# iwa-shi/CRDR

Measured on AMD Instinct MI355X. Metric: stage-3 training img/s at 256x256, higher is better.
Workload: dtype fp32; 1 GPU; config/crdr_stage_3.yaml -b 16: full GAN step (G + 5x CLIC21GVAE D + LPIPS-Alex, random-init weights), rate index cycled 0..4; global_batch=16, crop=256, parallelism=dp1

## Files before the change

crdr_amd/csrc/eltwise.hip:

```cpp

#include <algorithm>
#include <cmath>

#include "common.hpp"

namespace crdr {

struct EbwdArgs {
  crdr_ebwd_desc d;
  crdr_ebwd_io io;
  float* partial;
  int rows_per_block;
};

__global__ __launch_bounds__(256) void ebwd_kernel(const EbwdArgs p) {
  __shared__ float red[4][4][64];
  const int tx = threadIdx.x & 63, ty = threadIdx.x >> 6;
  const int f = p.d.flags, C = p.d.C;
  const int64_t r0 = (int64_t)blockIdx.x * p.rows_per_block;
  const int64_t r1 = r0 + p.rows_per_block < p.d.M ? r0 + p.rows_per_block : p.d.M;
  for (int c0 = 0; c0 < C; c0 += 64) {
    const int c = c0 + tx;
    float s0 = 0.f, s1 = 0.f, s2 = 0.f, s3 = 0.f;
    if (c < C) {
      const float sc = (f & CRDR_EPI_AFFINE) ? p.io.scale[c] : 1.f;
      const float sh = (f & CRDR_EPI_AFFINE) ? p.io.shift[c] : 0.f;
      const float v2 = (f & CRDR_EPI_VEC2) ? p.io.vec2[c] : 0.f;
      for (int64_t m = r0 + ty; m < r1; m += 4) {
        float g = p.io.dout[m * p.d.lddout + c];
        float o = (f & (CRDR_EPI_AFFINE | CRDR_EPI_RELU | CRDR_EPI_LRELU)) ? p.io.out[m * p.d.ldout + c] : 0.f;
        if (f & CRDR_EPI_AFFINE) {
          const float u = (o - sh) / sc;
          s2 += g * u;
          s3 += g;
          g *= sc;
          o = u;
        }
        if (f & CRDR_EPI_GATE) {
          const float sg = p.io.sig[m * p.d.ldg + c], tr = p.io.gt[m * p.d.ldg + c];
          p.io.gres[m * p.d.ldgres + c] = g;
          p.io.dgt[m * p.d.ldg + c] = g * sg;
          g = g * tr * sg * (1.f - sg);
        } else if ((f & CRDR_EPI_AFFINE) && (f & CRDR_EPI_RES)) {
          p.io.gres[m * p.d.ldgres + c] = g;
        }
        if (f & CRDR_EPI_VEC2) s1 += g;
        if (f & CRDR_EPI_RELU) g = (o - v2) > 0.f ? g : 0.f;
        if (f & CRDR_EPI_LRELU) g = o > 0.f ? g : 0.2f * g;
        if (p.io.dz) p.io.dz[m * p.d.lddz + c] = g;
        s0 += g;
      }
    }
    red[0][ty][tx] = s0; red[1][ty][tx] = s1; red[2][ty][tx] = s2; red[3][ty][tx] = s3;
    __syncthreads();
    if (ty == 0 && c < C) {
#pragma unroll
      for (int k = 0; k < 4; ++k)
        p.partial[((size_t)blockIdx.x * 4 + k) * C + c] = red[k][0][tx] + red[k][1][tx] + red[k][2][tx] + red[k][3][tx];
    }
    __syncthreads();
  }
}

__global__ __launch_bounds__(256) void ebwd_kernel_narrow(const EbwdArgs p) {
  __shared__ float red[16][256];
  const int f = p.d.flags, C = p.d.C, tid = threadIdx.x;
  const int64_t r0 = (int64_t)blockIdx.x * p.rows_per_block;
  const int64_t r1 = r0 + p.rows_per_block < p.d.M ? r0 + p.rows_per_block : p.d.M;
  float s[4][4];
  float sc[4], sh[4], v2[4];
#pragma unroll
  for (int c = 0; c < 4; ++c) {
    const bool live = c < C;
    sc[c] = (live && (f & CRDR_EPI_AFFINE)) ? p.io.scale[c] : 1.f;
    sh[c] = (live && (f & CRDR_EPI_AFFINE)) ? p.io.shift[c] : 0.f;
    v2[c] = (live && (f & CRDR_EPI_VEC2)) ? p.io.vec2[c] : 0.f;
#pragma unroll
    for (int k = 0; k < 4; ++k) s[k][c] = 0.f;
  }
  const bool need_out = f & (CRDR_EPI_AFFINE | CRDR_EPI_RELU | CRDR_EPI_LRELU);
  for (int64_t m = r0 + tid; m < r1; m += 256) {
#pragma unroll
    for (int c = 0; c < 4; ++c) {
      if (c >= C) continue;
      float g = p.io.dout[m * p.d.lddout + c];
      float o = need_out ? p.io.out[m * p.d.ldout + c] : 0.f;
      if (f & CRDR_EPI_AFFINE) {
// ... 190 lines not shown
      b += src[((size_t)sl * 2 + 1) * jb.cpad];
    }
    red[0][ty][tx] = a; red[1][ty][tx] = b;
    __syncthreads();
    if (ty == 0 && c < jb.C) {
      const float sa = ((red[0][0][tx] + red[0][1][tx]) + red[0][2][tx]) + red[0][3][tx];
      const float sb = ((red[1][0][tx] + red[1][1][tx]) + red[1][2][tx]) + red[1][3][tx];
      if (jb.out_pre) jb.out_pre[c] = jb.accumulate ? jb.out_pre[c] + sa : sa;
      if (jb.out_post) jb.out_post[c] = jb.accumulate ? jb.out_post[c] + sb : sb;
    }
    __syncthreads();
  }
}

static int ebwd_blocks(int64_t M, int* rpb) {
  int r = 64;
  while (cdiv64(M, r) > 512) r *= 2;
  *rpb = r;
  return (int)cdiv64(M, r);
}

__global__ __launch_bounds__(256) void affine_kernel(const float* x, int ldx, const float* scale, const float* shift,
                                                     float* y, int ldy, int64_t M, int C) {
  const int64_t total = M * C;
  for (int64_t e = blockIdx.x * 256ll + threadIdx.x; e < total; e += gridDim.x * 256ll) {
    const int64_t m = e / C;
    const int c = (int)(e - m * C);
    y[m * ldy + c] = x[m * ldx + c] * scale[c] + shift[c];
  }
}

__global__ __launch_bounds__(256) void add_affine_kernel(const float* a, int lda, const float* r, int ldr, const float* scale, const float* shift,
                                                         float* y, int ldy, int64_t M, int C4) {
  const int64_t total = M * C4;
  for (int64_t e = blockIdx.x * 256ll + threadIdx.x; e < total; e += gridDim.x * 256ll) {
    const int64_t m = e / C4;
    const int c = (int)(e - m * C4) * 4;
    f32x4 v = *reinterpret_cast<const f32x4*>(a + m * lda + c) + *reinterpret_cast<const f32x4*>(r + m * ldr + c);
    if (scale) v = v * *reinterpret_cast<const f32x4*>(scale + c) + *reinterpret_cast<const f32x4*>(shift + c);
    *reinterpret_cast<f32x4*>(y + m * ldy + c) = v;
  }
}

__global__ __launch_bounds__(256) void colsum_kernel(const float* x, int ldx, int64_t M, int C, float* partial,
                                                     int rows_per_block) {
  __shared__ float red[4][64];
  const int tx = threadIdx.x & 63, ty = threadIdx.x >> 6;
  const int64_t r0 = (int64_t)blockIdx.x * rows_per_block;
  const int64_t r1 = r0 + rows_per_block < M ? r0 + rows_per_block : M;
  for (int c0 = 0; c0 < C; c0 += 64) {
    const int c = c0 + tx;
    float s = 0.f;
    if (c < C)
      for (int64_t m = r0 + ty; m < r1; m += 4) s += x[m * ldx + c];
    red[ty][tx] = s;
    __syncthreads();
    if (ty == 0 && c < C) partial[(size_t)blockIdx.x * C + c] = red[0][tx] + red[1][tx] + red[2][tx] + red[3][tx];
    __syncthreads();
  }
}

__global__ __launch_bounds__(256) void colsum_kernel_v4(const float* x, int ldx, int64_t M, int C, float* partial,
                                                        int rows_per_block) {
  __shared__ f32x4 red[16][16];
  const int tx = threadIdx.x & 15, ty = threadIdx.x >> 4;
  const int c = blockIdx.y * 64 + tx * 4;
  const int64_t r0 = (int64_t)blockIdx.x * rows_per_block;
  const int64_t r1 = r0 + rows_per_block < M ? r0 + rows_per_block : M;
  f32x4 s = {0.f, 0.f, 0.f, 0.f};
  if (c < C)
    for (int64_t m = r0 + ty; m < r1; m += 16) s += *reinterpret_cast<const f32x4*>(x + m * ldx + c);
  red[ty][tx] = s;
  __syncthreads();
  if (threadIdx.x < 16 && c < C) {
    f32x4 a = red[0][tx];
#pragma unroll
    for (int r = 1; r < 16; ++r) a += red[r][tx];
    *reinterpret_cast<f32x4*>(partial + (size_t)blockIdx.x * C + c) = a;
  }
}

__device__ __forceinline__ float softplusf_(float w) { return w > 20.f ? w : log1pf(expf(w)); }

__global__ void interp_ca_params_kernel(const float* W, const float* B, int L, int C, float q, float* scale,
                                        float* shift) {
  const int c = blockIdx.x * blockDim.x + threadIdx.x;
  if (c >= C) return;
  const float lf = floorf(q);
  const float rf = fminf(lf + 1.f, (float)(L - 1));
  const float a = rf - q;
  const int l = (int)lf, r = (int)rf;
  const float w = W[l * C + c] * a + W[r * C + c] * (1.f - a);
  scale[c] = softplusf_(w);
  shift[c] = B ? B[l * C + c] * a + B[r * C + c] * (1.f - a) : 0.f;
}

__global__ void interp_ca_params_bwd_kernel(const float* W, int L, int C, float q, const float* dscale,
                                            const float* dshift, float* dW, float* dB) {
  const int c = blockIdx.x * blockDim.x + threadIdx.x;
  if (c >= C) return;
  const float lf = floorf(q);
  const float rf = fminf(lf + 1.f, (float)(L - 1));
  const float a = rf - q;
  const int l = (int)lf, r = (int)rf;
  const float w = W[l * C + c] * a + W[r * C + c] * (1.f - a);
  const float dw = dscale[c] * (w > 20.f ? 1.f : 1.f / (1.f + expf(-w)));
  dW[l * C + c] += dw * a;
  dW[r * C + c] += dw * (1.f - a);
  if (dB) {
    dB[l * C + c] += dshift[c] * a;
    dB[r * C + c] += dshift[c] * (1.f - a);
  }
}

__global__ __launch_bounds__(256) void lrp_kernel(const float* a, int lda, const float* z, int ldz, float* y, int ldy,
                                                  int64_t M, int C) {
  const int64_t total = M * C;
  for (int64_t e = blockIdx.x * 256ll + threadIdx.x; e < total; e += gridDim.x * 256ll) {
    const int64_t m = e / C;
    const int c = (int)(e - m * C);
    y[m * ldy + c] = a[m * lda + c] + 0.5f * tanhf(z[m * ldz + c]);
  }
}
__global__ __launch_bounds__(256) void lrp_bwd_kernel(const float* dy, int lddy, const float* z, int ldz, float* dz,
                                                      int lddz, int64_t M, int C) {
  const int64_t total = M * C;
  for (int64_t e = blockIdx.x * 256ll + threadIdx.x; e < total; e += gridDim.x * 256ll) {
    const int64_t m = e / C;
    const int c = (int)(e - m * C);
    const float t = tanhf(z[m * ldz + c]);
    dz[m * lddz + c] = dy[m * lddy + c] * 0.5f * (1.f - t * t);
  }
}

__global__ __launch_bounds__(256) void tanh_fwd_kernel(const float* x, int ldx, int64_t M, int C, int C4, float* y, int ldy) {
  const int64_t total = M * C4;
  for (int64_t e = blockIdx.x * 256ll + threadIdx.x; e < total; e += gridDim.x * 256ll) {
    const int64_t m = e / C4;
    const int c = (int)(e - m * C4) * 4;
    const f32x4 v = *reinterpret_cast<const f32x4*>(x + m * ldx + c);
    f32x4 o;
#pragma unroll
    for (int k = 0; k < 4; ++k) o[k] = c + k < C ? tanhf(v[k]) : 0.f;
    *reinterpret_cast<f32x4*>(y + m * ldy + c) = o;
  }
}
__global__ __launch_bounds__(256) void tanh_bwd_kernel(const float* y, int ldy, const float* dy, int lddy, int64_t M, int C, int C4,
                                                       float* dx, int lddx) {
  const int64_t total = M * C4;
  for (int64_t e = blockIdx.x * 256ll + threadIdx.x; e < total; e += gridDim.x * 256ll) {
    const int64_t m = e / C4;
    const int c = (int)(e - m * C4) * 4;
    const f32x4 t = *reinterpret_cast<const f32x4*>(y + m * ldy + c);
    const f32x4 g = *reinterpret_cast<const f32x4*>(dy + m * lddy + c);
    f32x4 o;
#pragma unroll
    for (int k = 0; k < 4; ++k) o[k] = c + k < C ? g[k] * (1.f - t[k] * t[k]) : 0.f;
    *reinterpret_cast<f32x4*>(dx + m * lddx + c) = o;
  }
}

__device__ __forceinline__ float block_sum_256(float v, float* red) {
#pragma unroll
  for (int o = 32; o > 0; o >>= 1) v += __shfl_down(v, o, 64);
  const int lane = threadIdx.x & 63, w = threadIdx.x >> 6;
  if (lane == 0) red[w] = v;
  __syncthreads();
  float r = red[0] + red[1] + red[2] + red[3];
  __syncthreads();
  return r;
}

enum { RED_SQDIFF = 0, RED_BCE = 1, RED_SQNORM = 2, RED_DOT = 3, RED_L1 = 4 };
template <int OP>
__global__ __launch_bounds__(256) void reduce_kernel(const float* a, const float* b, int64_t n, float target,
                                                     float* partial) {
  __shared__ float red[4];
  float s = 0.f;
  for (int64_t e = blockIdx.x * 256ll + threadIdx.x; e < n; e += gridDim.x * 256ll) {
    if (OP == RED_SQDIFF) { const float d = a[e] - b[e]; s += d * d; }
    if (OP == RED_L1) s += fabsf(a[e] - b[e]);
    if (OP == RED_SQNORM) { const float d = a[e]; s += d * d; }
    if (OP == RED_DOT) s += a[e] * b[e];
    if (OP == RED_BCE) {
      const float x = a[e] - b[e];
      s += fmaxf(x, 0.f) - x * target + log1pf(expf(-fabsf(x)));
    }
  }
  s = block_sum_256(s, red);
  if (threadIdx.x == 0) partial[blockIdx.x] = s;
}
__global__ __launch_bounds__(256) void reduce_final(const float* partial, int nb, float* out) {
  __shared__ float red[4];
  float s = 0.f;
  for (int e = threadIdx.x; e < nb; e += 256) s += partial[e];
  s = block_sum_256(s, red);
  if (threadIdx.x == 0) out[0] = s;
}
static int reduce_blocks(int64_t n) { return (int)std::min<int64_t>(std::max<int64_t>(cdiv64(n, 1024), 1), 1024); }

__global__ __launch_bounds__(256) void sqdiff_bwd_kernel(const float* a, const float* b, int64_t n, const float* g,
                                                         float gscale, float* da, float* db) {
  const float k = 2.f * gscale * (g ? g[0] : 1.f);
  for (int64_t e = blockIdx.x * 256ll + threadIdx.x; e < n; e += gridDim.x * 256ll) {
    const float d = (a[e] - b[e]) * k;
    if (da) da[e] = d;
    if (db) db[e] = -d;
  }
}
__global__ __launch_bounds__(256) void l1_bwd_kernel(const float* a, const float* b, int64_t n, const float* g, float gscale,
                                                     float* da, float* db) {
  const float k = gscale * (g ? g[0] : 1.f);
  for (int64_t e = blockIdx.x * 256ll + threadIdx.x; e < n; e += gridDim.x * 256ll) {
    const float x = a[e] - b[e];
    const float d = x > 0.f ? k : x < 0.f ? -k : 0.f;
    if (da) da[e] = d;
    if (db) db[e] = -d;
  }
}
__global__ __launch_bounds__(256) void bce_diff_bwd_kernel(const float* p, const float* q, int64_t n, float target,
                                                           const float* g, float gscale, float* dp, float* dq) {
  const float k = gscale * (g ? g[0] : 1.f);
  for (int64_t e = blockIdx.x * 256ll + threadIdx.x; e < n; e += gridDim.x * 256ll) {
    const float x = p[e] - q[e];
    const float d = (1.f / (1.f + expf(-x)) - target) * k;
    if (dp) dp[e] = d;
    if (dq) dq[e] = -d;
  }
}

__global__ __launch_bounds__(256) void adam_kernel(float* p, const float* g, float* m, float* v, int64_t n, float lr,
                                                   float b1, float b2, float eps, float bc1, float bc2_sqrt,
                                                   const float* sqnorm, float max_norm) {
  float clip = 1.f;
  if (sqnorm) {
    const float c = max_norm / (sqrtf(sqnorm[0]) + 1e-6f);
    clip = c < 1.f ? c : 1.f;
  }
  const float step_size = lr / bc1;
  for (int64_t e = blockIdx.x * 256ll + threadIdx.x; e < n; e += gridDim.x * 256ll) {
    const float gr = g[e] * clip;
    const float mm = m[e] + (gr - m[e]) * (1.f - b1);
    const float vv = v[e] * b2 + (1.f - b2) * gr * gr;
    m[e] = mm;
    v[e] = vv;
    const float denom = sqrtf(vv) / bc2_sqrt + eps;
    p[e] -= step_size * (mm / denom);
  }
}

__global__ __launch_bounds__(256) void adam_dyn_kernel(float* p, const float* g, float* m, float* v, int64_t n, float b1,
                                                       float b2, float eps, const float* dyn, const float* sqnorm,
                                                       float max_norm) {
  if (dyn[2] != 0.f) return;
  const float st = dyn[1];
  const float bc1 = 1.f - powf(b1, st), bc2_sqrt = sqrtf(1.f - powf(b2, st));
  float clip = 1.f;
  if (sqnorm) {
    const float c = max_norm / (sqrtf(sqnorm[0]) + 1e-6f);
    clip = c < 1.f ? c : 1.f;
  }
  const float step_size = dyn[0] / bc1;
  const bool vec = ((reinterpret_cast<uintptr_t>(p) | reinterpret_cast<uintptr_t>(g) | reinterpret_cast<uintptr_t>(m) | reinterpret_cast<uintptr_t>(v)) & 15) == 0;
  const int64_t n4 = vec ? n >> 2 : 0;
  for (int64_t e4 = blockIdx.x * 256ll + threadIdx.x; e4 < n4; e4 += gridDim.x * 256ll) {
    const f32x4 gv = reinterpret_cast<const f32x4*>(g)[e4], mv = reinterpret_cast<const f32x4*>(m)[e4], vv4 = reinterpret_cast<const f32x4*>(v)[e4];
    f32x4 pv = reinterpret_cast<const f32x4*>(p)[e4], mo, vo;
#pragma unroll
    for (int k = 0; k < 4; ++k) {
      const float gr = gv[k] * clip;
      const float mm = mv[k] + (gr - mv[k]) * (1.f - b1);
      const float vv = vv4[k] * b2 + (1.f - b2) * gr * gr;
      mo[k] = mm;
      vo[k] = vv;
      pv[k] -= step_size * (mm / (sqrtf(vv) / bc2_sqrt + eps));
    }
    reinterpret_cast<f32x4*>(m)[e4] = mo;
    reinterpret_cast<f32x4*>(v)[e4] = vo;
    reinterpret_cast<f32x4*>(p)[e4] = pv;
  }
  for (int64_t e = (n4 << 2) + blockIdx.x * 256ll + threadIdx.x; e < n; e += gridDim.x * 256ll) {
    const float gr = g[e] * clip;
    const float mm = m[e] + (gr - m[e]) * (1.f - b1);
    const float vv = v[e] * b2 + (1.f - b2) * gr * gr;
    m[e] = mm;
    v[e] = vv;
    p[e] -= step_size * (mm / (sqrtf(vv) / bc2_sqrt + eps));
  }
}

__global__ __launch_bounds__(256) void maxpool3s2_fwd_kernel(const float* x, float* y, int N, int H, int W, int C,
                                                             int OH, int OW) {
  const unsigned total = (unsigned)N * OH * OW * C;
  for (unsigned e = blockIdx.x * 256u + threadIdx.x; e < total; e += gridDim.x * 256u) {
    unsigned r = e / (unsigned)C;
    const int c = (int)(e - r * C);
    unsigned q = r / (unsigned)OW;
    const int ow = (int)(r - q * OW);
    const int n = (int)(q / (unsigned)OH), oh = (int)(q - (unsigned)n * OH);
    float best = -INFINITY;
    for (int i = 0; i < 3; ++i)
      for (int j = 0; j < 3; ++j) {
        const int ih = oh * 2 + i, iw = ow * 2 + j;
        if (ih < H && iw < W) best = fmaxf(best, x[(((int64_t)n * H + ih) * W + iw) * C + c]);
      }
    y[e] = best;
  }
}
__global__ __launch_bounds__(256) void maxpool3s2_bwd_kernel(const float* x, const float* dy, float* dx, int N, int H,
                                                             int W, int C, int OH, int OW) {
  const unsigned total = (unsigned)N * H * W * C;
  for (unsigned e = blockIdx.x * 256u + threadIdx.x; e < total; e += gridDim.x * 256u) {
    unsigned r = e / (unsigned)C;
    const int c = (int)(e - r * C);
    unsigned q = r / (unsigned)W;
    const int iw = (int)(r - q * W);
    const int n = (int)(q / (unsigned)H), ih = (int)(q - (unsigned)n * H);
    float acc = 0.f;
    for (int oh = (ih >= 2 ? (ih - 1) / 2 : 0); oh <= ih / 2 && oh < OH; ++oh)
      for (int ow = (iw >= 2 ? (iw - 1) / 2 : 0); ow <= iw / 2 && ow < OW; ++ow) {
        float best = -INFINITY; int bi = -1, bj = -1;
        for (int i = 0; i < 3; ++i)
          for (int j = 0; j < 3; ++j) {
            const int yy = oh * 2 + i, xx = ow * 2 + j;
            if (yy < H && xx < W) {
              const float v = x[(((int64_t)n * H + yy) * W + xx) * C + c];
              if (v > best) { best = v; bi = yy; bj = xx; }
            }
          }
        if (bi == ih && bj == iw) acc += dy[(((int64_t)n * OH + oh) * OW + ow) * C + c];
      }
    dx[e] = acc;
  }
}

__global__ __launch_bounds__(256) void lpips_layer_fwd_kernel(const float* f0, const float* f1, const float* lin,
                                                              int N, int HW, int C, float* partial) {
  __shared__ float red[4];
  const int lane = threadIdx.x & 63, w = threadIdx.x >> 6;
  const int n = blockIdx.y;
  float acc = 0.f;
  for (int px = blockIdx.x * 4 + w; px < HW; px += gridDim.x * 4) {
    const float* a = f0 + ((size_t)n * HW + px) * C;
    const float* b = f1 + ((size_t)n * HW + px) * C;
    float sa = 0.f, sb = 0.f;
    for (int c = lane; c < C; c += 64) { sa += a[c] * a[c]; sb += b[c] * b[c]; }
#pragma unroll
    for (int o = 32; o > 0; o >>= 1) { sa += __shfl_xor(sa, o, 64); sb += __shfl_xor(sb, o, 64); }
    const float ia = 1.f / (sqrtf(sa) + 1e-10f), ib = 1.f / (sqrtf(sb) + 1e-10f);
    float d = 0.f;
    for (int c = lane; c < C; c += 64) { const float t = a[c] * ia - b[c] * ib; d += lin[c] * t * t; }
#pragma unroll
    for (int o = 32; o > 0; o >>= 1) d += __shfl_xor(d, o, 64);
    acc += d;
  }
  if (lane == 0) red[w] = acc;
  __syncthreads();
  if (threadIdx.x == 0) partial[(size_t)n * gridDim.x + blockIdx.x] = red[0] + red[1] + red[2] + red[3];
}
__global__ void lpips_layer_final(const float* partial, int nb, int HW, float* out) {
  const int n = blockIdx.x;
  if (threadIdx.x == 0) {
    float s = 0.f;
    for (int b = 0; b < nb; ++b) s += partial[(size_t)n * nb + b];
    out[n] += s / (float)HW;
  }
}
__global__ __launch_bounds__(256) void lpips_layer_bwd_kernel(const float* f0, const float* f1, const float* lin,
                                                              int N, int HW, int C, const float* gout, float* df1) {
  const int lane = threadIdx.x & 63, w = threadIdx.x >> 6;
  const int n = blockIdx.y;
  const float g = gout[n] / (float)HW;
  for (int px = blockIdx.x * 4 + w; px < HW; px += gridDim.x * 4) {
    const float* a = f0 + ((size_t)n * HW + px) * C;
    const float* b = f1 + ((size_t)n * HW + px) * C;
    float* d = df1 + ((size_t)n * HW + px) * C;
    float sa = 0.f, sb = 0.f;
    for (int c = lane; c < C; c += 64) { sa += a[c] * a[c]; sb += b[c] * b[c]; }
#pragma unroll
    for (int o = 32; o > 0; o >>= 1) { sa += __shfl_xor(sa, o, 64); sb += __shfl_xor(sb, o, 64); }
    const float nb_ = sqrtf(sb);
    const float ia = 1.f / (sqrtf(sa) + 1e-10f), ib = 1.f / (nb_ + 1e-10f);
    float dot = 0.f;
    for (int c = lane; c < C; c += 64) {
      const float e = -2.f * g * lin[c] * (a[c] * ia - b[c] * ib);
      dot += e * b[c];
    }
#pragma unroll
    for (int o = 32; o > 0; o >>= 1) dot += __shfl_xor(dot, o, 64);
// ... 425 lines not shown
extern "C" int crdr_add_affine(const float* a, int lda, const float* r, int ldr, const float* scale, const float* shift, float* y, int ldy,
                               int64_t M, int C, crdr_stream_t s) {
  CRDR_REQUIRE(a && r && y && (!scale == !shift), "add_affine: null pointer (scale and shift come together)");
  CRDR_REQUIRE(M >= 0 && C > 0 && C % 4 == 0 && lda % 4 == 0 && ldr % 4 == 0 && ldy % 4 == 0 && lda >= C && ldr >= C && ldy >= C,
               "add_affine: C (%d) and the strides (%d, %d, %d) must be multiples of 4, the strides at least C", C, lda, ldr, ldy);
  CRDR_REQUIRE(((reinterpret_cast<uintptr_t>(a) | reinterpret_cast<uintptr_t>(r) | reinterpret_cast<uintptr_t>(y) |
                 reinterpret_cast<uintptr_t>(scale) | reinterpret_cast<uintptr_t>(shift)) & 15) == 0, "add_affine: operands must be 16-byte aligned");
  if (M == 0) return 0;
  hipLaunchKernelGGL(add_affine_kernel, dim3(grid_for(M * (C / 4))), dim3(256), 0, as_stream(s), a, lda, r, ldr, scale, shift, y, ldy, M, C / 4);
  CRDR_CHECK_LAUNCH("add_affine");
  return 0;
}

extern "C" size_t crdr_colsum_workspace(int64_t M, int C) {
  int rpb;
  return (size_t)ebwd_blocks(M, &rpb) * C * sizeof(float);
}
extern "C" int crdr_colsum(const float* x, int ldx, int64_t M, int C, float* out, int accumulate, void* ws,
                           size_t ws_bytes, crdr_stream_t s) {
  int rpb;
  const int nb = ebwd_blocks(M, &rpb);
  CRDR_REQUIRE(x && out && ws_bytes >= (size_t)nb * C * sizeof(float), "colsum: bad arguments");
  if (M > 0) {
    if ((C % 4 == 0) && (ldx % 4 == 0) && ((reinterpret_cast<uintptr_t>(x) & 15) == 0))
      hipLaunchKernelGGL(colsum_kernel_v4, dim3(nb, cdiv(C, 64)), dim3(256), 0, as_stream(s), x, ldx, M, C, (float*)ws, rpb);
    else
      hipLaunchKernelGGL(colsum_kernel, dim3(nb), dim3(256), 0, as_stream(s), x, ldx, M, C, (float*)ws, rpb);
    CRDR_CHECK_LAUNCH("colsum");
  }
  hipLaunchKernelGGL(colsum_final, dim3(cdiv(C, 16)), dim3(256), 0, as_stream(s), (const float*)ws, M > 0 ? nb : 0, 1,
                     C, out, accumulate, (float*)nullptr);
  CRDR_CHECK_LAUNCH("colsum_final");
  return 0;
}

extern "C" int crdr_colsum_slab_rows(void) { return kColsumSlab; }

extern "C" int crdr_colsum_finish_batched(const crdr_colsum_job* jobs, const int64_t* prefix_a, const int64_t* prefix_b,
                                          const int64_t* meta, float* scratch, crdr_stream_t s) {
  CRDR_REQUIRE(jobs && prefix_a && prefix_b && meta && scratch, "colsum_finish_batched: null pointer");
  hipLaunchKernelGGL(colsum_finish_a_kernel, dim3(4096), dim3(256), 0, as_stream(s), jobs, reinterpret_cast<const long long*>(prefix_a),
                     reinterpret_cast<const long long*>(meta), scratch);
  CRDR_CHECK_LAUNCH("colsum_finish_a_kernel");
  hipLaunchKernelGGL(colsum_finish_b_kernel, dim3(512), dim3(256), 0, as_stream(s), jobs, reinterpret_cast<const long long*>(prefix_b),
                     reinterpret_cast<const long long*>(meta), (const float*)scratch);
  CRDR_CHECK_LAUNCH("colsum_finish_b_kernel");
  return 0;
}

extern "C" int crdr_colsum_scatter(const float* x, int ldx, int64_t M, int C, int block, float* const* outs, int accumulate,
                                   void* ws, size_t ws_bytes, crdr_stream_t s) {
  int rpb;
  const int nb = ebwd_blocks(M, &rpb);
  CRDR_REQUIRE(x && outs && block > 0 && ws_bytes >= (size_t)nb * C * sizeof(float), "colsum_scatter: bad arguments");
  if (M > 0) {
    if ((C % 4 == 0) && (ldx % 4 == 0) && ((reinterpret_cast<uintptr_t>(x) & 15) == 0))
      hipLaunchKernelGGL(colsum_kernel_v4, dim3(nb, cdiv(C, 64)), dim3(256), 0, as_stream(s), x, ldx, M, C, (float*)ws, rpb);
    else
      hipLaunchKernelGGL(colsum_kernel, dim3(nb), dim3(256), 0, as_stream(s), x, ldx, M, C, (float*)ws, rpb);
    CRDR_CHECK_LAUNCH("colsum");
  }
  hipLaunchKernelGGL(colsum_final_scatter, dim3(cdiv(C, 16)), dim3(256), 0, as_stream(s), (const float*)ws, M > 0 ? nb : 0, C,
                     block, outs, accumulate);
  CRDR_CHECK_LAUNCH("colsum_final_scatter");
  return 0;
}

extern "C" int crdr_interp_ca_params(const float* W, const float* B, int L, int C, float q, float* scale,
                                     float* shift, crdr_stream_t s) {
  CRDR_REQUIRE(W && scale && shift, "interp_ca_params: null pointer");
  CRDR_REQUIRE(q >= 0.f && q <= (float)(L - 1), "interp_ca_params: rate_ind %f outside [0, %d]", q, L - 1);
  hipLaunchKernelGGL(interp_ca_params_kernel, dim3(cdiv(C, 64)), dim3(64), 0, as_stream(s), W, B, L, C, q, scale, shift);
  CRDR_CHECK_LAUNCH("interp_ca_params");
  return 0;
}
extern "C" int crdr_interp_ca_params_bwd(const float* W, int L, int C, float q, const float* dscale,
                                         const float* dshift, float* dW, float* dB, crdr_stream_t s) {
  CRDR_REQUIRE(W && dscale && dW, "interp_ca_params_bwd: null pointer");
  hipLaunchKernelGGL(interp_ca_params_bwd_kernel, dim3(cdiv(C, 64)), dim3(64), 0, as_stream(s), W, L, C, q, dscale,
                     dshift, dW, dB);
  CRDR_CHECK_LAUNCH("interp_ca_params_bwd");
  return 0;
}

extern "C" int crdr_lrp(const float* a, int lda, const float* z, int ldz, float* y, int ldy, int64_t M, int C,
                        crdr_stream_t s) {
  CRDR_REQUIRE(a && z && y, "lrp: null pointer");
  if (M * C == 0) return 0;
  hipLaunchKernelGGL(lrp_kernel, dim3(grid_for(M * C)), dim3(256), 0, as_stream(s), a, lda, z, ldz, y, ldy, M, C);
  CRDR_CHECK_LAUNCH("lrp");
  return 0;
}
extern "C" int crdr_lrp_bwd(const float* dy, int lddy, const float* z, int ldz, float* dz, int lddz, int64_t M, int C,
                            crdr_stream_t s) {
  CRDR_REQUIRE(dy && z && dz, "lrp_bwd: null pointer");
  if (M * C == 0) return 0;
  hipLaunchKernelGGL(lrp_bwd_kernel, dim3(grid_for(M * C)), dim3(256), 0, as_stream(s), dy, lddy, z, ldz, dz, lddz, M, C);
  CRDR_CHECK_LAUNCH("lrp_bwd");
  return 0;
}

static bool tanh_operand_ok(const float* p, int ld, int C) {
  return p && (reinterpret_cast<uintptr_t>(p) & 15) == 0 && ld % 4 == 0 && ld >= round_up(C, 4);
}
extern "C" int crdr_tanh_fwd(const float* x, int ldx, int64_t M, int C, float* y, int ldy, crdr_stream_t s) {
  CRDR_REQUIRE(M >= 0 && C > 0, "tanh_fwd: M (%lld) and C (%d) out of range", (long long)M, C);
  CRDR_REQUIRE(tanh_operand_ok(x, ldx, C) && tanh_operand_ok(y, ldy, C),
               "tanh_fwd: operands are 16-byte aligned, their strides multiples of 4 and at least C rounded up to 4");
  CRDR_REQUIRE(x != y || ldx == ldy, "tanh_fwd: in place needs one stride");
  if (M == 0) return 0;
  const int C4 = round_up(C, 4) / 4;
  hipLaunchKernelGGL(tanh_fwd_kernel, dim3(grid_for(M * C4)), dim3(256), 0, as_stream(s), x, ldx, M, C, C4, y, ldy);
  CRDR_CHECK_LAUNCH("tanh_fwd");
  return 0;
}
extern "C" int crdr_tanh_bwd(const float* y, int ldy, const float* dy, int lddy, int64_t M, int C, float* dx, int lddx, crdr_stream_t s) {
  CRDR_REQUIRE(M >= 0 && C > 0, "tanh_bwd: M (%lld) and C (%d) out of range", (long long)M, C);
  CRDR_REQUIRE(tanh_operand_ok(y, ldy, C) && tanh_operand_ok(dy, lddy, C) && tanh_operand_ok(dx, lddx, C),
               "tanh_bwd: operands are 16-byte aligned, their strides multiples of 4 and at least C rounded up to 4");
  CRDR_REQUIRE(dy != dx || lddy == lddx, "tanh_bwd: in place needs one stride");
  if (M == 0) return 0;
  const int C4 = round_up(C, 4) / 4;
  hipLaunchKernelGGL(tanh_bwd_kernel, dim3(grid_for(M * C4)), dim3(256), 0, as_stream(s), y, ldy, dy, lddy, M, C, C4, dx, lddx);
  CRDR_CHECK_LAUNCH("tanh_bwd");
  return 0;
}

struct BiasReluArgs {
  float* a;
  long long M;
  int ld, C, n;
  int c0[CRDR_MAX_GROUP];
  const float* bias[CRDR_MAX_GROUP];
};
__global__ __launch_bounds__(256) void bias_relu_slots_kernel(const BiasReluArgs p) {
  const int C4 = p.C >> 2;
  const long long per = p.M * C4, total = per * p.n;
  for (long long e = blockIdx.x * 256ll + threadIdx.x; e < total; e += gridDim.x * 256ll) {
    const int k = (int)(e / per);
    const long long r = e - k * per;
    const long long m = r / C4;
    const int c = (int)(r - m * C4) << 2;
    float* q = p.a + m * p.ld + p.c0[k] + c;
    const f32x4 v = *reinterpret_cast<const f32x4*>(q);
    const float* b = p.bias[k] + c;
    f32x4 o;
#pragma unroll
    for (int j = 0; j < 4; ++j) o[j] = fmaxf(v[j] + b[j], 0.f);
    *reinterpret_cast<f32x4*>(q) = o;
  }
}

extern "C" int crdr_bias_relu_slots(float* a, int ld, int64_t M, int C, int n, const int32_t* c0, const float* const* bias, crdr_stream_t s) {
  CRDR_REQUIRE(a && c0 && bias, "bias_relu_slots: null pointer");
  CRDR_REQUIRE(n >= 1 && n <= CRDR_MAX_GROUP && C % 4 == 0 && ld % 4 == 0 && (reinterpret_cast<uintptr_t>(a) & 15) == 0,
               "bias_relu_slots: %d slots of %d channels (ld %d)", n, C, ld);
  if (M * C == 0) return 0;
  BiasReluArgs p;
  p.a = a; p.M = M; p.ld = ld; p.C = C; p.n = n;
  for (int k = 0; k < n; ++k) {
    CRDR_REQUIRE(bias[k] && c0[k] % 4 == 0, "bias_relu_slots: slot %d misaligned", k);
    p.c0[k] = c0[k]; p.bias[k] = bias[k];
  }
  hipLaunchKernelGGL(bias_relu_slots_kernel, dim3(grid_for(M * (C / 4) * n)), dim3(256), 0, as_stream(s), p);
  CRDR_CHECK_LAUNCH("bias_relu_slots");
  return 0;
}

extern "C" size_t crdr_reduce_workspace(int64_t n) { return (size_t)reduce_blocks(n) * sizeof(float); }

template <int OP>
static int run_reduce(const float* a, const float* b, int64_t n, float target, float* out, void* ws, size_t ws_bytes,
                      crdr_stream_t s, const char* what) {
  const int nb = reduce_blocks(n);
  CRDR_REQUIRE(a && out && ws_bytes >= (size_t)nb * sizeof(float), "%s: bad arguments", what);
  hipLaunchKernelGGL(reduce_kernel<OP>, dim3(nb), dim3(256), 0, as_stream(s), a, b, n, target, (float*)ws);
  CRDR_CHECK_LAUNCH(what);
  hipLaunchKernelGGL(reduce_final, dim3(1), dim3(256), 0, as_stream(s), (const float*)ws, nb, out);
  CRDR_CHECK_LAUNCH(what);
  return 0;
}
extern "C" int crdr_spectral_norm_fwd(const float* w, int O, int K, float* u, float* v, int power_iter, float eps, float* w_out,
                                      float* sigma_out, void* ws, size_t ws_bytes, crdr_stream_t s) {
  CRDR_REQUIRE(w && u && v && w_out && sigma_out && ws, "spectral_norm_fwd: null pointer");
  CRDR_REQUIRE(ws_bytes >= (size_t)(O + K + 2) * sizeof(float), "spectral_norm_fwd: workspace too small");
  float* tv = (float*)ws;
  float* tu = tv + K;
  hipStream_t st = as_stream(s);
  if (power_iter) {
    hipLaunchKernelGGL(sn_wt_u_kernel, dim3(cdiv(K, 256)), dim3(256), 0, st, w, u, O, K, tv);
    hipLaunchKernelGGL(sn_normalize_kernel, dim3(1), dim3(1024), 0, st, tv, K, eps, v, 1, (float*)nullptr);
  }
  hipLaunchKernelGGL(sn_w_v_kernel, dim3(cdiv(O, 4)), dim3(256), 0, st, w, v, O, K, tu);
  hipLaunchKernelGGL(sn_normalize_kernel, dim3(1), dim3(1024), 0, st, tu, O, eps, u, power_iter ? 1 : 0, sigma_out);
  hipLaunchKernelGGL(sn_scale_kernel, dim3(grid_for((int64_t)O * K)), dim3(256), 0, st, w, sigma_out, (long long)O * K, w_out);
  CRDR_CHECK_LAUNCH("spectral_norm_fwd");
  return 0;
}

extern "C" int crdr_spectral_norm_bwd(const float* dw_sn, const float* w, const float* u, const float* v, const float* sigma,
                                      int O, int K, float* dw, void* ws, size_t ws_bytes, crdr_stream_t s) {
  CRDR_REQUIRE(dw_sn && w && u && v && sigma && dw && ws, "spectral_norm_bwd: null pointer");
  const int64_t n = (int64_t)O * K;
  const int nb = reduce_blocks(n);
  CRDR_REQUIRE(ws_bytes >= (size_t)(nb + 1) * sizeof(float), "spectral_norm_bwd: workspace too small");
  float* part = (float*)ws;
  float* dot = part + nb;
  hipStream_t st = as_stream(s);
  hipLaunchKernelGGL(reduce_kernel<RED_DOT>, dim3(nb), dim3(256), 0, st, dw_sn, w, n, 0.f, part);
  hipLaunchKernelGGL(reduce_final, dim3(1), dim3(256), 0, st, (const float*)part, nb, dot);
  hipLaunchKernelGGL(sn_bwd_kernel, dim3(grid_for(n)), dim3(256), 0, st, dw_sn, u, v, sigma, (const float*)dot, O, K, dw);
  CRDR_CHECK_LAUNCH("spectral_norm_bwd");
  return 0;
}

extern "C" int crdr_sqdiff_sum(const float* a, const float* b, int64_t n, float* out, void* ws, size_t ws_bytes,
                               crdr_stream_t s) {
  CRDR_REQUIRE(b, "sqdiff_sum: null pointer");
  return run_reduce<RED_SQDIFF>(a, b, n, 0.f, out, ws, ws_bytes, s, "sqdiff_sum");
}
extern "C" int crdr_l1_sum(const float* a, const float* b, int64_t n, float* out, void* ws, size_t ws_bytes, crdr_stream_t s) {
  CRDR_REQUIRE(b, "l1_sum: null pointer");
  return run_reduce<RED_L1>(a, b, n, 0.f, out, ws, ws_bytes, s, "l1_sum");
}
extern "C" int crdr_bce_diff_sum(const float* p, const float* q, int64_t n, float target, float* out, void* ws,
                                 size_t ws_bytes, crdr_stream_t s) {
  CRDR_REQUIRE(q, "bce_diff_sum: null pointer");
  return run_reduce<RED_BCE>(p, q, n, target, out, ws, ws_bytes, s, "bce_diff_sum");
}
extern "C" int crdr_sqnorm(const float* g, int64_t n, float* out, void* ws, size_t ws_bytes, crdr_stream_t s) {
  return run_reduce<RED_SQNORM>(g, nullptr, n, 0.f, out, ws, ws_bytes, s, "sqnorm");
}
extern "C" int crdr_sqdiff_bwd(const float* a, const float* b, int64_t n, const float* g, float gscale, float* da,
                               float* db, crdr_stream_t s) {
  CRDR_REQUIRE(a && b, "sqdiff_bwd: null pointer");
  if (n == 0) return 0;
  hipLaunchKernelGGL(sqdiff_bwd_kernel, dim3(grid_for(n)), dim3(256), 0, as_stream(s), a, b, n, g, gscale, da, db);
  CRDR_CHECK_LAUNCH("sqdiff_bwd");
  return 0;
}
extern "C" int crdr_l1_bwd(const float* a, const float* b, int64_t n, const float* g, float gscale, float* da, float* db,
                           crdr_stream_t s) {
  CRDR_REQUIRE(a && b, "l1_bwd: null pointer");
  if (n == 0) return 0;
  hipLaunchKernelGGL(l1_bwd_kernel, dim3(grid_for(n)), dim3(256), 0, as_stream(s), a, b, n, g, gscale, da, db);
  CRDR_CHECK_LAUNCH("l1_bwd");
  return 0;
}
extern "C" int crdr_bce_diff_bwd(const float* p, const float* q, int64_t n, float target, const float* g, float gscale,
                                 float* dp, float* dq, crdr_stream_t s) {
  CRDR_REQUIRE(p && q, "bce_diff_bwd: null pointer");
  if (n == 0) return 0;
  hipLaunchKernelGGL(bce_diff_bwd_kernel, dim3(grid_for(n)), dim3(256), 0, as_stream(s), p, q, n, target, g, gscale, dp, dq);
  CRDR_CHECK_LAUNCH("bce_diff_bwd");
  return 0;
}

extern "C" int crdr_adam_step(float* p, const float* g, float* m, float* v, int64_t n, float lr, float beta1,
                              float beta2, float eps, int step, const float* sqnorm, float max_norm, crdr_stream_t s) {
  CRDR_REQUIRE(p && g && m && v && step >= 1, "adam_step: bad arguments");
  if (n == 0) return 0;
  const float bc1 = 1.f - powf(beta1, (float)step);
  const float bc2_sqrt = sqrtf(1.f - powf(beta2, (float)step));
  hipLaunchKernelGGL(adam_kernel, dim3(grid_for(n)), dim3(256), 0, as_stream(s), p, g, m, v, n, lr, beta1, beta2, eps,
                     bc1, bc2_sqrt, sqnorm, max_norm);
  CRDR_CHECK_LAUNCH("adam_step");
  return 0;
}

extern "C" int crdr_adam_step_dyn(float* p, const float* g, float* m, float* v, int64_t n, float beta1, float beta2,
                                  float eps, const float* dyn, const float* sqnorm, float max_norm, crdr_stream_t s) {
  CRDR_REQUIRE(p && g && m && v && dyn, "adam_step_dyn: bad arguments");
  if (n == 0) return 0;
  hipLaunchKernelGGL(adam_dyn_kernel, dim3(grid_for(n)), dim3(256), 0, as_stream(s), p, g, m, v, n, beta1, beta2, eps, dyn,
                     sqnorm, max_norm);
  CRDR_CHECK_LAUNCH("adam_step_dyn");
  return 0;
}

extern "C" int crdr_maxpool3s2_fwd(const float* x, float* y, int N, int H, int W, int C, crdr_stream_t s) {
  CRDR_REQUIRE(x && y && H >= 3 && W >= 3, "maxpool: bad arguments");
  CRDR_REQUIRE((long long)N * H * W * C < (1ll << 31), "maxpool: %lld elements (32-bit element index)", (long long)N * H * W * C);
  const int OH = (H - 3) / 2 + 1, OW = (W - 3) / 2 + 1;
  hipLaunchKernelGGL(maxpool3s2_fwd_kernel, dim3(grid_for((int64_t)N * OH * OW * C)), dim3(256), 0, as_stream(s), x, y, N,
                     H, W, C, OH, OW);
  CRDR_CHECK_LAUNCH("maxpool_fwd");
  return 0;
}
extern "C" int crdr_maxpool3s2_bwd(const float* x, const float* dy, float* dx, int N, int H, int W, int C,
                                   crdr_stream_t s) {
  CRDR_REQUIRE(x && dy && dx && H >= 3 && W >= 3, "maxpool_bwd: bad arguments");
  CRDR_REQUIRE((long long)N * H * W * C < (1ll << 31), "maxpool_bwd: %lld elements (32-bit element index)", (long long)N * H * W * C);
  const int OH = (H - 3) / 2 + 1, OW = (W - 3) / 2 + 1;
  hipLaunchKernelGGL(maxpool3s2_bwd_kernel, dim3(grid_for((int64_t)N * H * W * C)), dim3(256), 0, as_stream(s), x, dy, dx,
                     N, H, W, C, OH, OW);
  CRDR_CHECK_LAUNCH("maxpool_bwd");
  return 0;
}

extern "C" int crdr_lpips_layer_fwd(const float* f0, const float* f1, const float* lin, int N, int HW, int C,
                                    float* out, void* ws, size_t ws_bytes, crdr_stream_t s) {
  CRDR_REQUIRE(f0 && f1 && lin && out && ws, "lpips_layer_fwd: bad arguments");
  const int nb = std::min(cdiv(HW, 4), 64);
  CRDR_REQUIRE(ws_bytes >= (size_t)N * nb * sizeof(float), "lpips_layer_fwd: workspace too small");
  float* part = (float*)ws;
  hipLaunchKernelGGL(lpips_layer_fwd_kernel, dim3(nb, N), dim3(256), 0, as_stream(s), f0, f1, lin, N, HW, C, part);
  CRDR_CHECK_LAUNCH("lpips_layer_fwd");
  hipLaunchKernelGGL(lpips_layer_final, dim3(N), dim3(64), 0, as_stream(s), (const float*)part, nb, HW, out);
  CRDR_CHECK_LAUNCH("lpips_layer_final");
  return 0;
}
extern "C" int crdr_lpips_layer_bwd(const float* f0, const float* f1, const float* lin, int N, int HW, int C,
                                    const float* gout, float* df1, crdr_stream_t s) {
  CRDR_REQUIRE(f0 && f1 && lin && gout && df1, "lpips_layer_bwd: bad arguments");
  const int nb = std::min(cdiv(HW, 4), 256);
  hipLaunchKernelGGL(lpips_layer_bwd_kernel, dim3(nb, N), dim3(256), 0, as_stream(s), f0, f1, lin, N, HW, C, gout, df1);
  CRDR_CHECK_LAUNCH("lpips_layer_bwd");
  return 0;
}
```

crdr_amd/csrc/entropy.hip:

```cpp

#include <algorithm>
#include <cmath>

#include "common.hpp"

namespace crdr {

__device__ __forceinline__ float exp_neg_sq(float x) {
  const float kL2Ehi = 1.44269502162933349609375f, kL2Elo = 1.92596299112661746e-8f;
  const float s = x * x, slo = __builtin_fmaf(x, x, -s);
  const float ti = __builtin_rintf(s * kL2Ehi);
  float tf = __builtin_fmaf(s, kL2Ehi, -ti);
  tf = __builtin_fmaf(s, kL2Elo, tf);
  tf = __builtin_fmaf(slo, kL2Ehi, tf);
  return __builtin_ldexpf(__builtin_amdgcn_exp2f(-tf), -(int)ti);
}
__device__ __forceinline__ float erfcx_pos(float a) {
  const float q = (a - 2.f) * __builtin_amdgcn_rcpf(a + 2.f);
  float p = 6.807514774e-05f;
  p = __builtin_fmaf(p, q, 1.608403462e-04f);
  p = __builtin_fmaf(p, q, -3.709284118e-04f);
  p = __builtin_fmaf(p, q, -1.395805088e-03f);
  p = __builtin_fmaf(p, q, 1.230503218e-03f);
  p = __builtin_fmaf(p, q, 8.689252695e-03f);
  p = __builtin_fmaf(p, q, -8.024739103e-03f);
  p = __builtin_fmaf(p, q, -5.421199524e-02f);
  p = __builtin_fmaf(p, q, 1.640504971e-01f);
  p = __builtin_fmaf(p, q, -1.660310904e-01f);
  p = __builtin_fmaf(p, q, -9.276381574e-02f);
  p = __builtin_fmaf(p, q, 2.769783912e-01f);
  const float r = __builtin_amdgcn_rcpf(__builtin_fmaf(2.f, a, 1.f));
  return __builtin_fmaf(p, r, r);
}
__device__ __forceinline__ float gc_rs(float sg) {
  const float r0 = __builtin_amdgcn_rcpf(sg);
  return __builtin_fmaf(__builtin_fmaf(-sg, r0, 1.f), r0, r0) * 0.70710678118654752440f;
}
__device__ __forceinline__ float gc_lik(float a, float rs, float& e_lo, float& e_hi) {
  const float xh = fminf((a + 0.5f) * rs, 1e4f), xl = fminf(fmaxf((a - 0.5f) * rs, -1e4f), 1e4f);
  e_hi = exp_neg_sq(xh);
  e_lo = exp_neg_sq(xl);
  const float th = e_hi * erfcx_pos(xh), tl = e_lo * erfcx_pos(fabsf(xl));
  const float l = 0.5f * ((xl < 0.f ? 2.f - tl : tl) - th);
  return a != a ? a : l;
}
__device__ __forceinline__ float gc_floor(float l, float bound) { return l < bound ? bound : l; }

__device__ __forceinline__ float block_sum(float v, float* red) {
#pragma unroll
  for (int o = 32; o > 0; o >>= 1) v += __shfl_down(v, o, 64);
  const int lane = threadIdx.x & 63, w = threadIdx.x >> 6, nw = blockDim.x >> 6;
  __syncthreads();
  if (lane == 0) red[w] = v;
  __syncthreads();
  float r = 0.f;
  for (int i = 0; i < nw; ++i) r += red[i];
  return r;
}

struct GcArgs {
  crdr_gc_desc2 d;
  crdr_gc_io io;
};

__device__ __forceinline__ void philox4x32_10(unsigned c0, unsigned c1, unsigned c2, unsigned c3, unsigned k0, unsigned k1,
                                              unsigned out[4]) {
#pragma unroll
  for (int r = 0; r < 10; ++r) {
    const unsigned hi0 = __umulhi(0xD2511F53u, c0), lo0 = 0xD2511F53u * c0;
    const unsigned hi1 = __umulhi(0xCD9E8D57u, c2), lo1 = 0xCD9E8D57u * c2;
    const unsigned n0 = hi1 ^ c1 ^ k0, n2 = hi0 ^ c3 ^ k1;
    c0 = n0; c1 = lo1; c2 = n2; c3 = lo0;
    k0 += 0x9E3779B9u; k1 += 0xBB67AE85u;
  }
  out[0] = c0; out[1] = c1; out[2] = c2; out[3] = c3;
}
__device__ __forceinline__ float philox_uniform(const uint64_t* ph, unsigned long long idx) {
  const unsigned long long seed = ph[0], ctr = ph[1] + (idx >> 2);
  unsigned o[4];
  philox4x32_10((unsigned)ctr, (unsigned)(ctr >> 32), 0u, 0u, (unsigned)seed, (unsigned)(seed >> 32), o);
  const unsigned r = o[idx & 3];
  return (float)(r >> 8) * (1.0f / 16777216.0f) - 0.5f;
}

__device__ __forceinline__ float gc_noise(const GcArgs& p, size_t pix, int c) {
  if (p.io.noise) return p.io.noise[pix * p.d.ldnoise + c];
  return philox_uniform(p.io.philox, (unsigned long long)pix * p.d.Ctot + p.d.c0 + c);
}

__device__ __forceinline__ void gc_elem(const GcArgs& p, float yv, float m, float sraw, float u, bool noisy, bool want_q, float& q_plus_m,
                                        float& lq, float& ln, float& sn, float& sq) {
  const float sg = fmaxf(sraw, p.d.scale_bound);
  const float rs = gc_rs(sg);
  const float q = rintf(yv - m);
  q_plus_m = q + m;
  float e0, e1;
  if (want_q) {
    float l = gc_lik(fabsf(q), rs, e0, e1);
    l = gc_floor(l, p.d.likelihood_bound);
    lq = l;
    sq -= __builtin_amdgcn_logf(l);
  }
  if (noisy) {
    float l = gc_lik(fabsf(yv + u - m), rs, e0, e1);
    l = gc_floor(l, p.d.likelihood_bound);
    ln = l;
    sn -= __builtin_amdgcn_logf(l);
  }
}

template <bool VEC>
__global__ __launch_bounds__(256) void gauss_cond_fwd_kernel(const GcArgs p, float* part) {
  __shared__ float red[16];
  const int n = blockIdx.y, C = p.d.C;
  const int per_img = p.d.HW * C;
  const bool noisy = p.io.noise || p.io.philox;
  const bool want_q = p.io.lik_quant || p.io.bits_quant;
  float sn = 0.f, sq = 0.f;
  if (VEC) {
    const int C4 = C >> 2;
    for (int e4 = blockIdx.x * 256 + threadIdx.x; e4 < (per_img >> 2); e4 += gridDim.x * 256) {
      const int px = e4 / C4, c = (e4 - px * C4) << 2;
      const size_t pix = (size_t)n * p.d.HW + px;
      const float4 yv = *reinterpret_cast<const float4*>(p.io.y + pix * p.d.ldy + c);
      const float4 mv = *reinterpret_cast<const float4*>(p.io.mu + pix * p.d.ldmu + c);
      const float4 sv = *reinterpret_cast<const float4*>(p.io.sigma + pix * p.d.ldsigma + c);
      float u[4] = {0.f, 0.f, 0.f, 0.f};
      if (p.io.noise) {
        const float4 nv = *reinterpret_cast<const float4*>(p.io.noise + pix * p.d.ldnoise + c);
        u[0] = nv.x; u[1] = nv.y; u[2] = nv.z; u[3] = nv.w;
      } else if (p.io.philox) {
        const unsigned long long idx = (unsigned long long)pix * p.d.Ctot + p.d.c0 + c;
        const unsigned long long seed = p.io.philox[0], ctr = p.io.philox[1] + (idx >> 2);
        unsigned o[4];
        philox4x32_10((unsigned)ctr, (unsigned)(ctr >> 32), 0u, 0u, (unsigned)seed, (unsigned)(seed >> 32), o);
#pragma unroll
        for (int j = 0; j < 4; ++j) u[j] = (float)(o[j] >> 8) * (1.0f / 16777216.0f) - 0.5f;
      }
      const float ya[4] = {yv.x, yv.y, yv.z, yv.w}, ma[4] = {mv.x, mv.y, mv.z, mv.w}, sa[4] = {sv.x, sv.y, sv.z, sv.w};
      float qm[4], lq[4], ln[4];
#pragma unroll
      for (int j = 0; j < 4; ++j) gc_elem(p, ya[j], ma[j], sa[j], u[j], noisy, want_q, qm[j], lq[j], ln[j], sn, sq);
      const float4 qv = make_float4(qm[0], qm[1], qm[2], qm[3]);
      if (p.io.yhat) *reinterpret_cast<float4*>(p.io.yhat + pix * p.d.ldyhat + c) = qv;
      if (p.io.yhat2) *reinterpret_cast<float4*>(p.io.yhat2 + pix * p.d.ldyhat2 + c) = qv;
      if (p.io.lik_quant) *reinterpret_cast<float4*>(p.io.lik_quant + pix * p.d.ldlik + c) = make_float4(lq[0], lq[1], lq[2], lq[3]);
      if (p.io.lik_noisy && noisy) *reinterpret_cast<float4*>(p.io.lik_noisy + pix * p.d.ldlik + c) = make_float4(ln[0], ln[1], ln[2], ln[3]);
    }
  } else {
    for (int e = blockIdx.x * 256 + threadIdx.x; e < per_img; e += gridDim.x * 256) {
      const int px = e / C, c = e - px * C;
      const size_t pix = (size_t)n * p.d.HW + px;
      float qm, lq = 0.f, ln = 0.f;
      gc_elem(p, p.io.y[pix * p.d.ldy + c], p.io.mu[pix * p.d.ldmu + c], p.io.sigma[pix * p.d.ldsigma + c],
              noisy ? gc_noise(p, pix, c) : 0.f, noisy, want_q, qm, lq, ln, sn, sq);
      if (p.io.yhat) p.io.yhat[pix * p.d.ldyhat + c] = qm;
      if (p.io.yhat2) p.io.yhat2[pix * p.d.ldyhat2 + c] = qm;
      if (p.io.lik_quant) p.io.lik_quant[pix * p.d.ldlik + c] = lq;
      if (p.io.lik_noisy && noisy) p.io.lik_noisy[pix * p.d.ldlik + c] = ln;
    }
  }
  sn = block_sum(sn, red);
  sq = block_sum(sq, red);
  if (threadIdx.x == 0) {
    if (part) {
      float* o = part + ((size_t)n * gridDim.x + blockIdx.x) * 2;
      o[0] = sn; o[1] = sq;
    } else {
      if (p.io.bits_noisy && noisy) p.io.bits_noisy[n] += sn;
      if (p.io.bits_quant) p.io.bits_quant[n] += sq;
    }
  }
}

__global__ __launch_bounds__(256) void gauss_cond_finish_kernel(const float* part, int B, float* bits_noisy, float* bits_quant) {
  __shared__ float red[16];
  const int n = blockIdx.x;
  float sn = 0.f, sq = 0.f;
  for (int b = threadIdx.x; b < B; b += 256) {
    const float2 v = *reinterpret_cast<const float2*>(part + ((size_t)n * B + b) * 2);
    sn += v.x; sq += v.y;
  }
  sn = block_sum(sn, red);
  sq = block_sum(sq, red);
  if (threadIdx.x == 0) {
    if (bits_noisy) bits_noisy[n] += sn;
    if (bits_quant) bits_quant[n] += sq;
  }
}

__device__ __forceinline__ void gc_elem_bwd(const GcArgs& p, float yv, float m, float sraw, float u, float gb, float ste, float& gy_out,
                                            float& gmu, float& gsig) {
  const float inv_ln2 = 1.4426950408889634f;
  const float sg = fmaxf(sraw, p.d.scale_bound);
  const float dlt = yv + u - m;
  const float a = fabsf(dlt), sgn = dlt > 0.f ? 1.f : (dlt < 0.f ? -1.f : 0.f);
  const float rs = gc_rs(sg), inv_sg = rs * 1.41421356237309504880f;
  const float zu = (0.5f - a) * inv_sg, zl = (-0.5f - a) * inv_sg;
  float e_lo, e_hi;
  const float lraw = gc_lik(a, rs, e_lo, e_hi);
  const float l = gc_floor(lraw, p.d.likelihood_bound);
  const float glik = gb * (-inv_ln2 / l);
  const float graw = (lraw < p.d.likelihood_bound && glik >= 0.f) ? 0.f : glik;
  const float pu = 0.39894228040143267794f * e_lo, pl = 0.39894228040143267794f * e_hi;
  const float dl_da = (pl - pu) * inv_sg;
  const float dl_dsg = (zl * pl - zu * pu) * inv_sg;
  const float gy = graw * dl_da * sgn;
  const float gsg = graw * dl_dsg;
  gsig = (sraw < p.d.scale_bound && gsg >= 0.f) ? 0.f : gsg;
  gy_out = gy + ste;
  gmu = -gy;
}

template <bool VEC>
__global__ __launch_bounds__(256) void gauss_cond_bwd_kernel(const GcArgs p) {
  const int C = p.d.C;
  const int per_img = p.d.HW * C;
  const int64_t total = (int64_t)p.d.N * per_img;
  if (VEC) {
    const int C4 = C >> 2;
    for (int64_t e4 = blockIdx.x * 256ll + threadIdx.x; e4 < (total >> 2); e4 += gridDim.x * 256ll) {
      const size_t pix = (size_t)(e4 / C4);
      const int c = (int)(e4 - (int64_t)pix * C4) << 2;
      const int n = (int)(pix / p.d.HW);
      const float4 yv = *reinterpret_cast<const float4*>(p.io.y + pix * p.d.ldy + c);
      const float4 mv = *reinterpret_cast<const float4*>(p.io.mu + pix * p.d.ldmu + c);
      const float4 sv = *reinterpret_cast<const float4*>(p.io.sigma + pix * p.d.ldsigma + c);
      float4 dv = make_float4(0.f, 0.f, 0.f, 0.f);
      if (p.io.dyhat) dv = *reinterpret_cast<const float4*>(p.io.dyhat + pix * p.d.lddyhat + c);
      float u[4];
      if (p.io.noise) {
        const float4 nv = *reinterpret_cast<const float4*>(p.io.noise + pix * p.d.ldnoise + c);
        u[0] = nv.x; u[1] = nv.y; u[2] = nv.z; u[3] = nv.w;
      } else {
        const unsigned long long idx = (unsigned long long)pix * p.d.Ctot + p.d.c0 + c;
        const unsigned long long seed = p.io.philox[0], ctr = p.io.philox[1] + (idx >> 2);
        unsigned o[4];
        philox4x32_10((unsigned)ctr, (unsigned)(ctr >> 32), 0u, 0u, (unsigned)seed, (unsigned)(seed >> 32), o);
#pragma unroll
        for (int j = 0; j < 4; ++j) u[j] = (float)(o[j] >> 8) * (1.0f / 16777216.0f) - 0.5f;
      }
      const float gb = p.io.gbits[n];
      const float ya[4] = {yv.x, yv.y, yv.z, yv.w}, ma[4] = {mv.x, mv.y, mv.z, mv.w}, sa[4] = {sv.x, sv.y, sv.z, sv.w};
      const float da[4] = {dv.x, dv.y, dv.z, dv.w};
      float gy[4], gm[4], gs[4];
#pragma unroll
      for (int j = 0; j < 4; ++j) gc_elem_bwd(p, ya[j], ma[j], sa[j], u[j], gb, da[j], gy[j], gm[j], gs[j]);
      *reinterpret_cast<float4*>(p.io.dy + pix * p.d.ldgrad + c) = make_float4(gy[0], gy[1], gy[2], gy[3]);
      *reinterpret_cast<float4*>(p.io.dmu + pix * p.d.ldgrad + c) = make_float4(gm[0], gm[1], gm[2], gm[3]);
      *reinterpret_cast<float4*>(p.io.dsigma + pix * p.d.ldgrad + c) = make_float4(gs[0], gs[1], gs[2], gs[3]);
    }
    return;
  }
  for (int64_t e = blockIdx.x * 256ll + threadIdx.x; e < total; e += gridDim.x * 256ll) {
    const int n = (int)(e / per_img);
    const size_t pix = (size_t)(e / C);
    const int c = (int)(e - (int64_t)pix * C);
    const float ste = p.io.dyhat ? p.io.dyhat[pix * p.d.lddyhat + c] : 0.f;
    float gy, gm, gs;
    gc_elem_bwd(p, p.io.y[pix * p.d.ldy + c], p.io.mu[pix * p.d.ldmu + c], p.io.sigma[pix * p.d.ldsigma + c], gc_noise(p, pix, c),
                p.io.gbits[n], ste, gy, gm, gs);
    p.io.dy[pix * p.d.ldgrad + c] = gy;
    p.io.dmu[pix * p.d.ldgrad + c] = gm;
    p.io.dsigma[pix * p.d.ldgrad + c] = gs;
  }
}

__global__ __launch_bounds__(256) void philox_uniform_kernel(const uint64_t* ph, int64_t M, int C, int Ctot, int c0, float* out, int ld) {
  const int64_t total = M * C;
  for (int64_t e = blockIdx.x * 256ll + threadIdx.x; e < total; e += gridDim.x * 256ll) {
    const int64_t pix = e / C;
// ... 139 lines not shown
    const float l = fmaxf(lraw, bound);
    const float glik = gbits[n] * (-inv_ln2 / l);
    const float graw = (lraw >= bound || glik < 0.f) ? glik : 0.f;
    const float sd = D > 0.f ? 1.f : (D < 0.f ? -1.f : 0.f);
    const float gu = graw * sd * A * (1.f - A) * s;
    const float gl = -graw * sd * B * (1.f - B) * s;
    float dx = eb_logits_bwd(P, v + 0.5f, Tu, gu, g);
    dx += eb_logits_bwd(P, v - 0.5f, Tl, gl, g);
    dz[idx] = dx + (dzhat ? dzhat[idx] : 0.f);
  }
  const int lane = threadIdx.x & 63, w = threadIdx.x >> 6;
#pragma unroll
  for (int i = 0; i < CRDR_EB_PARAMS; ++i) {
    float v = g[i];
#pragma unroll
    for (int o = 32; o > 0; o >>= 1) v += __shfl_down(v, o, 64);
    if (lane == 0) red[w][i] = v;
  }
  __syncthreads();
  if (threadIdx.x < CRDR_EB_PARAMS) {
    const int i = threadIdx.x;
    dparams[(size_t)c * CRDR_EB_PARAMS + i] = red[0][i] + red[1][i] + red[2][i] + red[3][i];
  }
}

__global__ __launch_bounds__(1024) void bits_kernel(const float* lik, int per_img, float* bits) {
  __shared__ float red[16];
  const int n = blockIdx.x;
  float s = 0.f;
  for (int e = threadIdx.x; e < per_img; e += blockDim.x) s -= logf(lik[(size_t)n * per_img + e]);
  s = block_sum(s, red);
  if (threadIdx.x == 0) bits[n] += s * 1.4426950408889634f;
}

__global__ __launch_bounds__(256) void eb_quantile_kernel(const float* quantiles, const float* params,
                                                          const float* target, int C, float* loss, float* dq) {
  __shared__ float red[16];
  float acc = 0.f;
  for (int e = threadIdx.x; e < C * 3; e += blockDim.x) {
    const int c = e / 3, j = e - c * 3;
    EbParams P;
    eb_load(params + (size_t)c * CRDR_EB_PARAMS, P);
    EbTape T;
    float g[CRDR_EB_PARAMS];
#pragma unroll
    for (int i = 0; i < CRDR_EB_PARAMS; ++i) g[i] = 0.f;
    const float x = quantiles[e];
    const float d = eb_logits(P, x, T) - target[j];
    const float sgn = d > 0.f ? 1.f : (d < 0.f ? -1.f : 0.f);
    acc += fabsf(d);
    dq[e] = eb_logits_bwd(P, x, T, sgn, g);
  }
  acc = block_sum(acc, red);
  if (threadIdx.x == 0) loss[0] = acc;
}

}

using namespace crdr;

extern "C" int crdr_eb_quantile_loss(const float* quantiles, const float* params, const float* target, int C,
                                     float* loss, float* dquantiles, crdr_stream_t s) {
  CRDR_REQUIRE(quantiles && params && target && loss && dquantiles, "eb_quantile_loss: null pointer");
  hipLaunchKernelGGL(eb_quantile_kernel, dim3(1), dim3(256), 0, as_stream(s), quantiles, params, target, C, loss,
                     dquantiles);
  CRDR_CHECK_LAUNCH("eb_quantile_loss");
  return 0;
}

static void gc_fill_defaults(crdr_gc_desc2& d) {
  if (!d.ldnoise) d.ldnoise = d.C;
  if (!d.ldlik) d.ldlik = d.C;
  if (!d.ldgrad) d.ldgrad = d.C;
  if (!d.Ctot) d.Ctot = d.C;
}

static int gc_blocks(const crdr_gc_desc2* d) {
  const long long per_img = (long long)d->HW * d->C;
  return (int)std::max<long long>(1, std::min<long long>(cdiv64(per_img, 1024), 2048));
}

extern "C" size_t crdr_gauss_cond_fwd_workspace(const crdr_gc_desc2* d) {
  if (!d) return 0;
  return (size_t)d->N * gc_blocks(d) * 2 * sizeof(float);
}

extern "C" int crdr_gauss_cond_fwd2(const crdr_gc_desc2* d, const crdr_gc_io* io, crdr_stream_t s) {
  CRDR_REQUIRE(d && io && io->y && io->mu && io->sigma, "gauss_cond_fwd: null input");
  GcArgs a;
  a.d = *d; a.io = *io;
  gc_fill_defaults(a.d);
  const long long per_img = (long long)d->HW * d->C;
  if (per_img == 0 || d->N == 0) return 0;
  CRDR_REQUIRE(per_img < (1ll << 31), "gauss_cond_fwd: %lld elements per image", per_img);
  auto al16 = [](const void* q) { return (reinterpret_cast<uintptr_t>(q) & 15) == 0; };
  const crdr_gc_desc2& g = a.d;
  const bool vec = g.C % 4 == 0 && g.ldy % 4 == 0 && g.ldmu % 4 == 0 && g.ldsigma % 4 == 0 && g.Ctot % 4 == 0 && g.c0 % 4 == 0 &&
                   al16(io->y) && al16(io->mu) && al16(io->sigma) && (!io->noise || (g.ldnoise % 4 == 0 && al16(io->noise))) &&
                   (!io->yhat || (g.ldyhat % 4 == 0 && al16(io->yhat))) && (!io->yhat2 || (g.ldyhat2 % 4 == 0 && al16(io->yhat2))) &&
                   ((!io->lik_noisy && !io->lik_quant) || (g.ldlik % 4 == 0 && al16(io->lik_noisy) && al16(io->lik_quant)));
  int B = gc_blocks(d);
  float* part = io->ws;
  if (!part || io->ws_bytes < crdr_gauss_cond_fwd_workspace(d) || !(io->bits_noisy || io->bits_quant)) {
    part = nullptr;
    if (io->bits_noisy || io->bits_quant) B = 1;
  }
  if (vec)
    hipLaunchKernelGGL(gauss_cond_fwd_kernel<true>, dim3(B, d->N), dim3(256), 0, as_stream(s), a, part);
  else
    hipLaunchKernelGGL(gauss_cond_fwd_kernel<false>, dim3(B, d->N), dim3(256), 0, as_stream(s), a, part);
  CRDR_CHECK_LAUNCH("gauss_cond_fwd");
  if (part) {
    const bool noisy = io->noise || io->philox;
    hipLaunchKernelGGL(gauss_cond_finish_kernel, dim3(d->N), dim3(256), 0, as_stream(s), part, B, noisy ? io->bits_noisy : nullptr,
                       io->bits_quant);
    CRDR_CHECK_LAUNCH("gauss_cond_finish");
  }
  return 0;
}

extern "C" int crdr_gauss_cond_bwd2(const crdr_gc_desc2* d, const crdr_gc_io* io, crdr_stream_t s) {
  CRDR_REQUIRE(d && io && io->y && io->mu && io->sigma && (io->noise || io->philox) && io->gbits && io->dy && io->dmu && io->dsigma,
               "gauss_cond_bwd: null pointer");
  GcArgs a;
  a.d = *d; a.io = *io;
  gc_fill_defaults(a.d);
  const int64_t total = (int64_t)d->N * d->HW * d->C;
  if (total == 0) return 0;
  auto al16 = [](const void* q) { return (reinterpret_cast<uintptr_t>(q) & 15) == 0; };
  const crdr_gc_desc2& g = a.d;
  const bool vec = g.C % 4 == 0 && g.ldy % 4 == 0 && g.ldmu % 4 == 0 && g.ldsigma % 4 == 0 && g.ldgrad % 4 == 0 && g.Ctot % 4 == 0 &&
                   g.c0 % 4 == 0 && al16(io->y) && al16(io->mu) && al16(io->sigma) && al16(io->dy) && al16(io->dmu) && al16(io->dsigma) &&
                   (!io->noise || (g.ldnoise % 4 == 0 && al16(io->noise))) && (!io->dyhat || (g.lddyhat % 4 == 0 && al16(io->dyhat)));
  const int nb = (int)std::min<int64_t>(cdiv64(vec ? total / 4 : total, 256), 4096);
  if (vec)
    hipLaunchKernelGGL(gauss_cond_bwd_kernel<true>, dim3(nb), dim3(256), 0, as_stream(s), a);
  else
    hipLaunchKernelGGL(gauss_cond_bwd_kernel<false>, dim3(nb), dim3(256), 0, as_stream(s), a);
  CRDR_CHECK_LAUNCH("gauss_cond_bwd");
  return 0;
}

__global__ __launch_bounds__(256) void gauss_symbols_kernel(const float* y, int ldy, const float* mu, int ldmu, const float* sigma,
                                                            int ldsg, const float* table, int levels, float bound, int N, int HW,
                                                            int C, int* sym, int* idx) {
  __shared__ float st[256];
  if (idx)
    for (int i = threadIdx.x; i < levels; i += 256) st[i] = table[i];
  __syncthreads();
  const long long total = (long long)N * C * HW;
  for (long long e = blockIdx.x * 256ll + threadIdx.x; e < total; e += gridDim.x * 256ll) {
    const int px = (int)(e % HW);
    const long long r = e / HW;
    const int c = (int)(r % C), n = (int)(r / C);
    const size_t pix = (size_t)n * HW + px;
    if (sym) sym[e] = (int)rintf(y[pix * ldy + c] - mu[pix * ldmu + c]);
    if (idx) {
      const float s = fmaxf(sigma[pix * ldsg + c], bound);
      int k = 0;
      for (int i = 0; i < levels - 1; ++i) k += (s > st[i]) ? 1 : 0;
      idx[e] = k;
    }
  }
}

extern "C" int crdr_gauss_symbols(const float* y, int ldy, const float* mu, int ldmu, const float* sigma, int ldsigma,
                                  const float* scale_table, int levels, float scale_bound, int N, int HW, int C, int32_t* symbols,
                                  int32_t* indexes, crdr_stream_t s) {
  CRDR_REQUIRE((!symbols || (y && mu)) && (!indexes || (sigma && scale_table)) && levels >= 1 && levels <= 256, "gauss_symbols: bad arguments");
  const long long total = (long long)N * C * HW;
  if (total == 0) return 0;
  hipLaunchKernelGGL(gauss_symbols_kernel, dim3((int)std::min<long long>(cdiv64(total, 256), 8192)), dim3(256), 0, as_stream(s), y, ldy, mu,
                     ldmu, sigma, ldsigma, scale_table, levels, scale_bound, N, HW, C, symbols, indexes);
  CRDR_CHECK_LAUNCH("gauss_symbols");
  return 0;
}

__global__ void philox_fork_kernel(uint64_t* state, uint64_t* call, unsigned long long inc) {
  call[0] = state[0];
  call[1] = state[1];
  state[1] += inc;
}

extern "C" int crdr_philox_fork(uint64_t* state, uint64_t* call, uint64_t inc, crdr_stream_t s) {
  CRDR_REQUIRE(state && call, "philox_fork: null pointer");
  hipLaunchKernelGGL(philox_fork_kernel, dim3(1), dim3(1), 0, as_stream(s), state, call, (unsigned long long)inc);
  CRDR_CHECK_LAUNCH("philox_fork");
  return 0;
}

extern "C" int crdr_philox_uniform(const uint64_t* philox, int N, int HW, int C, int Ctot, int c0, float* out, int ld,
                                   crdr_stream_t s) {
  CRDR_REQUIRE(philox && out, "philox_uniform: null pointer");
  const int64_t M = (int64_t)N * HW, total = M * C;
  if (total == 0) return 0;
// ... 60 lines not shown
```

crdr_amd/hip/functional.py:

```python
from __future__ import annotations

import ctypes as C
from typing import Optional, Tuple

import torch

from . import lib as L
from . import ops, packs

def grad_slot(p: torch.Tensor) -> torch.Tensor:
    if p.grad is None:
        p.grad = torch.zeros_like(p, memory_format=torch.contiguous_format)
    return p.grad


class ConvSpec:

    def __init__(self, in_ch, out_ch, k, stride, pad, transposed=False, out_pad=0):
        self.in_ch, self.out_ch, self.k = in_ch, out_ch, (k, k) if isinstance(k, int) else tuple(k)
        self.stride, self.pad, self.transposed, self.out_pad = stride, pad, transposed, out_pad
        self._packs = {}
        self.smallc = (not transposed) and in_ch <= 4
        self.smallc_dgrad = transposed and out_ch <= 4

# ... 225 lines not shown
            and x.shape[3] == 1 and x.shape[0] <= 16 and vec2 is None and res is None and affine is None and gate is None
            and act in (None, "relu") and weight.is_contiguous()):
        return _SmallLinear.apply(x, weight, bias, act == "relu")
    scale, shift = affine if affine is not None else (None, None)
    gx, gt = gate if gate is not None else (None, None)
    return _FusedConv.apply(x, weight, bias, vec2, res, scale, shift, gx, gt, spec, act, return_wgrad)


class _SpectralNorm(torch.autograd.Function):

    @staticmethod
    def forward(ctx, w_orig, u, v, training: bool, out_buf: torch.Tensor, eps: float):
        lib = L.load()
        ops._require_gpu(w_orig)
        o, k = w_orig.shape[0], w_orig.numel() // w_orig.shape[0]
        sigma = torch.empty(1, dtype=torch.float32, device=w_orig.device)
        ws, wsn = ops.workspace((o + k + 2) * 4, w_orig.device)
        L.check(lib.crdr_spectral_norm_fwd(w_orig.data_ptr(), o, k, u.data_ptr(), v.data_ptr(), int(training), float(eps),
                                           out_buf.data_ptr(), sigma.data_ptr(), ws, wsn, ops._stream()), "spectral_norm_fwd")
        ctx.save_for_backward(w_orig, u.clone() if training else u, v.clone() if training else v, sigma)
        return out_buf.detach()

    @staticmethod
    def backward(ctx, dw_sn):
        w_orig, u, v, sigma = ctx.saved_tensors
        lib = L.load()
        o, k = w_orig.shape[0], w_orig.numel() // w_orig.shape[0]
        g = grad_slot(w_orig)
        nb = lib.crdr_reduce_workspace(o * k) + 16
        ws, wsn = ops.workspace(nb, w_orig.device)
        L.check(lib.crdr_spectral_norm_bwd(dw_sn.contiguous().data_ptr(), w_orig.data_ptr(), u.data_ptr(), v.data_ptr(),
                                           sigma.data_ptr(), o, k, g.data_ptr(), ws, wsn, ops._stream()), "spectral_norm_bwd")
        return None, None, None, None, None, None


def spectral_norm_weight(w_orig, u, v, training: bool, out_buf: torch.Tensor, eps: float = 1e-12):
    return _SpectralNorm.apply(w_orig, u, v, training, out_buf, eps)


class _InterpCaVectors(torch.autograd.Function):
    @staticmethod
    def forward(ctx, W, B, q: float):
        lib = L.load()
        Lv, Cc = W.shape[0], W.shape[2]
        scale = torch.empty(Cc, dtype=torch.float32, device=W.device)
        shift = torch.empty(Cc, dtype=torch.float32, device=W.device)
        L.check(lib.crdr_interp_ca_params(W.data_ptr(), None if B is None else B.data_ptr(), Lv, Cc, float(q),
                                          scale.data_ptr(), shift.data_ptr(), ops._stream()), "interp_ca_params")
        ctx.q, ctx.has_b = float(q), B is not None
        ctx.B = B
        ctx.save_for_backward(W)
        return scale, shift

    @staticmethod
    def backward(ctx, dscale, dshift):
        (W,) = ctx.saved_tensors
        lib = L.load()
        Lv, Cc = W.shape[0], W.shape[2]
        direct = W.is_leaf and (ctx.B is None or ctx.B.is_leaf)
        if direct:
            dW = grad_slot(W) if ctx.needs_input_grad[0] else None
            dB = grad_slot(ctx.B) if (ctx.has_b and ctx.needs_input_grad[1]) else None
        else:
            dW = torch.zeros_like(W)
            dB = torch.zeros_like(W) if ctx.has_b else None
        if dW is not None or dB is not None:
            scratch = None
            if dW is None:
                scratch = dW = torch.zeros_like(W)
            L.check(lib.crdr_interp_ca_params_bwd(W.data_ptr(), Lv, Cc, ctx.q, dscale.contiguous().data_ptr(),
                                                  dshift.contiguous().data_ptr(), dW.data_ptr(),
                                                  None if dB is None else dB.data_ptr(), ops._stream()), "interp_ca_params_bwd")
            if scratch is not None:
                dW = None
        if direct:
            return None, None, None
        return dW, dB, None


def interp_ca_vectors(W, B, q: float):
    return _InterpCaVectors.apply(W, B, float(q))


class _Affine(torch.autograd.Function):
    @staticmethod
    def forward(ctx, x, scale, shift):
        lib = L.load()
        x, ld = ops.nhwc(x)
        n, c, h, w = x.shape
        y = ops.empty_nhwc(n, c, h, w, x.device)
        L.check(lib.crdr_affine(x.data_ptr(), ld, scale.data_ptr(), shift.data_ptr(), y.data_ptr(), ops.ld_for(c), n * h * w, c,
                                ops._stream()), "affine")
        ctx.save_for_backward(y, scale, shift)
        return y

    @staticmethod
    def backward(ctx, dy):
        y, scale, shift = ctx.saved_tensors
        dz, _, _, cs = ops.epilogue_bwd(dy, y, L.EPI_AFFINE, scale=scale, shift=shift)
        return dz, cs[2], cs[3]


def affine(x, scale, shift):
    return _Affine.apply(x, scale, shift)


class _AddAffine(torch.autograd.Function):

    @staticmethod
    def forward(ctx, a, r, scale, shift):
        lib = L.load()
        a, lda = ops.nhwc(a)
        r, ldr = ops.nhwc(r)
        if a.shape != r.shape:
            raise L.CrdrHipError(f"add_affine: operands of shapes {tuple(a.shape)} and {tuple(r.shape)}")
        n, c, h, w = a.shape
        y = ops.empty_nhwc(n, c, h, w, a.device)
        L.check(lib.crdr_add_affine(a.data_ptr(), lda, r.data_ptr(), ldr, ops._p(scale), ops._p(shift), y.data_ptr(), ops.ld_for(c), n * h * w, c,
                                    ops._stream()), "add_affine")
        ctx.save_for_backward(*((y, scale, shift) if scale is not None else ()))
        return y

    @staticmethod
    def backward(ctx, dy):
        if not ctx.saved_tensors:
            return dy, dy, None, None
        y, scale, shift = ctx.saved_tensors
        dz, _, _, cs = ops.epilogue_bwd(dy, y, L.EPI_AFFINE, scale=scale, shift=shift)
        return dz, dz, cs[2], cs[3]


def add_affine(a, r, affine: Optional[Tuple[torch.Tensor, torch.Tensor]] = None):
    scale, shift = affine if affine is not None else (None, None)
    return _AddAffine.apply(a, r, scale, shift)


class _PixelShuffle(torch.autograd.Function):

    @staticmethod
    def forward(ctx, x):
        lib = L.load()
        x, ldx = ops.nhwc(x)
        n, c4, h, w = x.shape
        if c4 % 4 != 0:
            raise L.CrdrHipError(f"pixel_shuffle: {c4} input channels are not a multiple of 4")
        c = c4 // 4
        y = ops.empty_nhwc(n, c, 2 * h, 2 * w, x.device)
        L.check(lib.crdr_pixel_shuffle_fwd(x.data_ptr(), ldx, n, h, w, c, y.data_ptr(), ops.ld_for(c), ops._stream()), "pixel_shuffle_fwd")
        ctx.in_shape = (n, c4, h, w)
        return y

    @staticmethod
    def backward(ctx, dy):
        lib = L.load()
        n, c4, h, w = ctx.in_shape
        dy, lddy = ops.nhwc(dy)
        dx = ops.empty_nhwc(n, c4, h, w, dy.device)
        L.check(lib.crdr_pixel_shuffle_bwd(dy.data_ptr(), lddy, n, h, w, c4 // 4, dx.data_ptr(), c4, ops._stream()), "pixel_shuffle_bwd")
        return dx


def pixel_shuffle(x):
    return _PixelShuffle.apply(x)


UPSAMPLE16_MODES = {"nearest": 0, "bilinear": 1, "bicubic": 2}
# ... 279 lines not shown
        return out

    @staticmethod
    def backward(ctx, g):
        fa, fb = ctx.saved_tensors
        lib = L.load()
        entry = _PAIR_SUMS[ctx.name][1]
        da = torch.empty_like(fa) if ctx.needs_input_grad[0] else None
        db = torch.empty_like(fb) if ctx.needs_input_grad[1] else None
        L.check(getattr(lib, "crdr_" + entry)(fa.data_ptr(), fb.data_ptr(), fa.numel(), *ctx.targs, g.contiguous().data_ptr(), 1.0,
                                              ops._p(da), ops._p(db), ops._stream()), entry)
        return _unflat(da, ctx.shapes[0], ctx.geom), _unflat(db, ctx.shapes[1], ctx.geom), None, None


def sqdiff_sum(a, b):
    return _PairSum.apply(a, b, "sqdiff_sum", None)


def l1_sum(a, b):
    return _PairSum.apply(a, b, "l1_sum", None)


def bce_diff_sum(p, q, target: float):
    return _PairSum.apply(p, q, "bce_diff_sum", float(target))


GAN_BCE, GAN_HINGE_D, GAN_HINGE_G = 0, 1, 2


class _GanLossSum(torch.autograd.Function):

    @staticmethod
    def forward(ctx, p, q, mask, kind, target, sgn, center):
        lib = L.load()
        fp = p.contiguous().reshape(-1)
        fq = None if q is None else q.contiguous().reshape(-1)
        fm = None if mask is None else mask.expand_as(p).contiguous().reshape(-1)
        if fq is not None and not center and fq.numel() != fp.numel():
            raise ValueError(f"gan_loss_sum: paired operands of {fp.numel()} and {fq.numel()} elements")
        if center and fq is None:
            raise ValueError("gan_loss_sum: center=True needs q")
        for t in (fp, fq, fm):
            if t is not None and (t.dtype != torch.float32 or t.device != p.device or not t.is_cuda):
                raise ValueError("gan_loss_sum: operands are float32 tensors on one GPU")
        d = L.GanLossDesc(n=fp.numel(), nq=0 if fq is None else fq.numel(), kind=int(kind), center=int(bool(center)),
                          target=float(target), sgn=float(sgn))
        out = torch.empty(1, dtype=torch.float32, device=p.device)
        stats = torch.empty(2, dtype=torch.float32, device=p.device)
        ws, wsn = ops.workspace(lib.crdr_gan_loss_workspace(d.n, d.nq), p.device)
        L.check(lib.crdr_gan_loss_fwd(C.byref(d), fp.data_ptr(), ops._p(fq), ops._p(fm), out.data_ptr(), stats.data_ptr(), ws, wsn,
                                      ops._stream()), "gan_loss_fwd")
        ctx.desc, ctx.has_q, ctx.has_mask = d, fq is not None, fm is not None
        ctx.shapes = (p.shape, None if q is None else q.shape)
        ctx.save_for_backward(fp, stats, *([fq] if fq is not None else []), *([fm] if fm is not None else []))
        return out

    @staticmethod
    def backward(ctx, g):
        lib = L.load()
        fp, stats, *rest = ctx.saved_tensors
        fq = rest.pop(0) if ctx.has_q else None
        fm = rest.pop(0) if ctx.has_mask else None
        d = ctx.desc
        dp = torch.empty_like(fp) if ctx.needs_input_grad[0] else None
        dq = torch.empty_like(fq) if (fq is not None and ctx.needs_input_grad[1]) else None
        ws, wsn = ops.workspace(lib.crdr_gan_loss_workspace(d.n, d.nq), fp.device)
        L.check(lib.crdr_gan_loss_bwd(C.byref(d), fp.data_ptr(), ops._p(fq), ops._p(fm), stats.data_ptr(), g.contiguous().data_ptr(), 1.0,
                                      ops._p(dp), ops._p(dq), ws, wsn, ops._stream()), "gan_loss_bwd")
        return (_unflat(dp, ctx.shapes[0], None), _unflat(dq, ctx.shapes[1], None), None, None, None, None, None)


def gan_loss_sum(p, q=None, *, kind: int, target: float = 0.0, sgn: float = 1.0, center: bool = False, mask=None):
    return _GanLossSum.apply(p, q, mask, int(kind), float(target), float(sgn), bool(center))


class _MaxPool3s2(torch.autograd.Function):
    @staticmethod
    def forward(ctx, x):
        lib = L.load()
        x = ops.dense_nhwc(x)
        n, c, h, w = x.shape
        oh, ow = (h - 3) // 2 + 1, (w - 3) // 2 + 1
        y = ops.empty_nhwc(n, c, oh, ow, x.device, ld=c)
        L.check(lib.crdr_maxpool3s2_fwd(x.data_ptr(), y.data_ptr(), n, h, w, c, ops._stream()), "maxpool_fwd")
        ctx.save_for_backward(x)
        return y

    @staticmethod
    def backward(ctx, dy):
        (x,) = ctx.saved_tensors
        lib = L.load()
        n, c, h, w = x.shape
        dy = ops.dense_nhwc(dy)
        dx = ops.empty_nhwc(n, c, h, w, x.device, ld=c)
        L.check(lib.crdr_maxpool3s2_bwd(x.data_ptr(), dy.data_ptr(), dx.data_ptr(), n, h, w, c, ops._stream()), "maxpool_bwd")
        return dx


def maxpool3s2(x):
    return _MaxPool3s2.apply(x)


class _LpipsLayer(torch.autograd.Function):

    @staticmethod
    def forward(ctx, f0, f1, lin):
        lib = L.load()
        f0, f1 = ops.dense_nhwc(f0), ops.dense_nhwc(f1)
        n, c, h, w = f0.shape
        out = torch.zeros(n, dtype=torch.float32, device=f0.device)
        ws, wsn = ops.workspace(n * 64 * 4, f0.device)
        L.check(lib.crdr_lpips_layer_fwd(f0.data_ptr(), f1.data_ptr(), lin.data_ptr(), n, h * w, c, out.data_ptr(), ws, wsn,
                                         ops._stream()), "lpips_layer_fwd")
        ctx.save_for_backward(f0, f1, lin)
        return out

    @staticmethod
    def backward(ctx, g):
        f0, f1, lin = ctx.saved_tensors
        lib = L.load()
        n, c, h, w = f0.shape
        df1 = ops.empty_nhwc(n, c, h, w, f0.device, ld=c)
        L.check(lib.crdr_lpips_layer_bwd(f0.data_ptr(), f1.data_ptr(), lin.data_ptr(), n, h * w, c, g.contiguous().data_ptr(),
                                         df1.data_ptr(), ops._stream()), "lpips_layer_bwd")
        return None, df1, None


def lpips_layer(f_real, f_fake, lin):
    return _LpipsLayer.apply(f_real, f_fake, lin)
```

crdr_amd/hip/lib.py:

```python
from __future__ import annotations

import ctypes as C
import os
import subprocess
import threading

_HERE = os.path.dirname(os.path.abspath(__file__))
CSRC_DIR = os.path.normpath(os.path.join(_HERE, "..", "csrc"))
LIB_PATH = os.environ.get("CRDR_HIP_LIB") or os.path.normpath(os.path.join(_HERE, "..", "_lib", "libcrdr_hip.so"))

c_float_p = C.POINTER(C.c_float)
c_void_p = C.c_void_p


class ConvDesc(C.Structure):
    _fields_ = [(n, C.c_int32) for n in (
        "N", "H", "W", "C", "OH", "OW", "OC", "kh", "kw", "stride", "pad", "transposed", "ldx", "ldy",
        "wrows", "wcols", "flags", "ldres", "ldg", "wlayout", "reserved", "ldpre", "ldmask")]


class ConvIO(C.Structure):
    _fields_ = [(n, c_void_p) for n in (
        "x", "w", "y", "bias", "vec2", "res", "scale", "shift", "gx", "gt", "sig", "pre", "mask", "cs")]


class ColsumJob(C.Structure):
    _fields_ = [("cs", c_void_p), ("out_pre", c_void_p), ("out_post", c_void_p)] + [(n, C.c_int32) for n in (
        "rows", "ld", "C", "accumulate", "nslab", "cpad")] + [("scratch_off", C.c_int64)]


class WgradDesc(C.Structure):
    _fields_ = [(n, C.c_int32) for n in (
        "N", "PH", "PW", "PC", "ldp", "QH", "QW", "QC", "ldq", "kh", "kw", "stride", "pad", "gI", "gJ",
        "accumulate", "algo")]


class EbwdDesc(C.Structure):
    _fields_ = [("M", C.c_int64)] + [(n, C.c_int32) for n in (
        "C", "flags", "lddout", "ldout", "lddz", "ldgres", "ldg")]


class WgradJob(C.Structure):
    _fields_ = [("slab", c_void_p), ("g", c_void_p)] + [(n, C.c_int32) for n in (
        "PC", "QC", "gI", "gJ", "T", "nsplit", "smallj", "accumulate", "gJtot", "reserved")]


class LinearGroup(C.Structure):
    _fields_ = [(n, c_void_p * 16) for n in ("w", "b", "y", "dy", "dw", "db")] + [("O", C.c_int32 * 16)]


class PackItem(C.Structure):
    _fields_ = [("src", c_void_p), ("dst", c_void_p)] + [(n, C.c_int32) for n in (
        "I", "J", "T", "rows", "cols", "mode", "srcJ", "dld")] + [("tstride", C.c_int64)]


class W4FilterItem(C.Structure):
    _fields_ = [("w", c_void_p * 16), ("u", c_void_p)] + [(n, C.c_int32) for n in (
        "G", "Cin", "Cout", "wrows", "wcols", "kchunks", "ntile", "nvar")] + [("widx", (C.c_int32 * 9) * 4), ("units", C.c_int64)]


class GdnDesc(C.Structure):
    _fields_ = [("M", C.c_int64)] + [(n, C.c_int32) for n in ("C", "ldx", "ldy", "inverse")] + [
        ("beta_min", C.c_float), ("reparam_offset", C.c_float)]


class ChannelNormDesc(C.Structure):
    _fields_ = [("M", C.c_int64)] + [(n, C.c_int32) for n in ("C", "ldx", "ldy", "ldres", "act")] + [
        ("slope", C.c_float), ("eps", C.c_float)]


class InstanceNormDesc(C.Structure):
    _fields_ = [("HW", C.c_int64)] + [(n, C.c_int32) for n in ("N", "C", "ldx", "ldy", "act")] + [("slope", C.c_float), ("eps", C.c_float)]


class GanLossDesc(C.Structure):
    _fields_ = [("n", C.c_int64), ("nq", C.c_int64), ("kind", C.c_int32), ("center", C.c_int32), ("target", C.c_float), ("sgn", C.c_float)]


class Upsample16Desc(C.Structure):
    _fields_ = [(n, C.c_int32) for n in ("N", "h", "w", "Cc", "ldi", "ldc", "ldo", "mode")]


class GcDesc2(C.Structure):
    _fields_ = [(n, C.c_int32) for n in ("N", "HW", "C", "ldy", "ldmu", "ldsigma", "ldyhat", "ldyhat2", "ldnoise", "ldlik",
                                         "ldgrad", "lddyhat", "Ctot", "c0")] + [
        ("scale_bound", C.c_float), ("likelihood_bound", C.c_float)]


class GcIO(C.Structure):
    _fields_ = [(n, c_void_p) for n in ("y", "mu", "sigma", "noise", "philox", "yhat", "yhat2", "lik_noisy", "lik_quant",
                                        "bits_noisy", "bits_quant", "gbits", "dyhat", "dy", "dmu", "dsigma", "ws")] + [
        ("ws_bytes", C.c_size_t)]


class EbwdIO(C.Structure):
    _fields_ = [(n, c_void_p) for n in (
        "dout", "out", "vec2", "scale", "shift", "gt", "sig", "dz", "gres", "dgt", "colsums", "dbias_accum")]


class GcDesc(C.Structure):
    _fields_ = [(n, C.c_int32) for n in ("N", "HW", "C", "ldy", "ldmu", "ldsigma", "ldyhat")] + [
        ("scale_bound", C.c_float), ("likelihood_bound", C.c_float)]


EPI_BIAS, EPI_RELU, EPI_LRELU, EPI_VEC2, EPI_RES, EPI_GATE, EPI_AFFINE, EPI_ACCUM = 1, 2, 4, 8, 16, 32, 64, 128
EPI_PREADD, EPI_RELUMASK, EPI_LRELUMASK, EPI_MASKOFF, EPI_COLSUM = 256, 512, 1024, 2048, 4096
CONV_NOSPLIT, CONV_BF16X3, WGRAD_BF16X3 = 8192, 16384, 1 << 16
CONV_BF16X6, WGRAD_BF16X6 = 32768, 1 << 17
WGRAD_SQUARE_Q = 1 << 18
MAX_GROUP = 16
EB_PARAMS = 58

_I, _I64, _F, _D, _P, _SZ = C.c_int, C.c_int64, C.c_float, C.c_double, c_void_p, C.c_size_t
SIGNATURES = {
    "crdr_last_error": (C.c_char_p, []),
    "crdr_version": (_I, []),
    "crdr_arch": (C.c_char_p, []),
    "crdr_profile_enable": (None, [_I]),
    "crdr_profile_read": (_I, [_I, C.POINTER(C.c_double), C.POINTER(C.c_double), C.POINTER(C.c_longlong)]),
    "crdr_conv2d_num_configs": (_I, []),
    "crdr_conv2d_num_stream_configs": (_I, []),
    "crdr_conv2d_num_wino_configs": (_I, []),
    "crdr_conv2d_wgrad_num_configs": (_I, []),
    "crdr_conv2d_wgrad_num_wino_configs": (_I, []),
    "crdr_conv2d_workspace": (_SZ, [C.POINTER(ConvDesc)]),
    "crdr_conv2d_choose_algo": (_I, [C.POINTER(ConvDesc), _I]),
    "crdr_conv2d": (_I, [C.POINTER(ConvDesc), C.POINTER(ConvIO), _P, _SZ, _P]),
    "crdr_conv2d_flops": (_D, [C.POINTER(ConvDesc)]),
    "crdr_conv2d_colsum_layout": (_I, [C.POINTER(ConvDesc), _I, C.POINTER(C.c_int), C.POINTER(C.c_int)]),
    "crdr_colsum_slab_rows": (_I, []),
    "crdr_colsum_finish_batched": (_I, [_P, _P, _P, _P, _P, _P]),
    "crdr_conv2d_grouped_workspace": (_SZ, [C.POINTER(ConvDesc), _I]),
    "crdr_conv2d_grouped": (_I, [C.POINTER(ConvDesc), _P, _I, _P, _SZ, _P]),
    "crdr_conv2d_filter_cache_bytes": (_SZ, [C.POINTER(ConvDesc), _I]),
    "crdr_conv2d_grouped_ex": (_I, [C.POINTER(ConvDesc), _P, _I, _P, _SZ, _P, _SZ, _I, _P]),
    "crdr_conv2d_filter_item": (_I, [C.POINTER(ConvDesc), _I, C.POINTER(W4FilterItem)]),
    "crdr_w4_filters_batched": (_I, [_P, _P, _P, _P]),
    "crdr_conv2d_wgrad_grouped_workspace": (_SZ, [C.POINTER(WgradDesc), _I]),
    "crdr_conv2d_wgrad_partial_grouped": (_I, [C.POINTER(WgradDesc), _P, _P, _P, _I, _P, _SZ, _P, _P]),
    "crdr_pack_weight_item": (_I, [C.POINTER(PackItem), _P]),
    "crdr_colsum_scatter": (_I, [_P, _I, _I64, _I, _I, _P, _I, _P, _SZ, _P]),
    "crdr_gauss_cond_fwd_workspace": (_SZ, [C.POINTER(GcDesc2)]),
    "crdr_gauss_cond_fwd2": (_I, [C.POINTER(GcDesc2), C.POINTER(GcIO), _P]),
    "crdr_gauss_cond_bwd2": (_I, [C.POINTER(GcDesc2), C.POINTER(GcIO), _P]),
    "crdr_gdn_workspace": (_SZ, [C.POINTER(GdnDesc), _I]),
    "crdr_gdn_fwd": (_I, [C.POINTER(GdnDesc), _P, _P, _P, _P, _P, _SZ, _P]),
    "crdr_gdn_bwd": (_I, [C.POINTER(GdnDesc), _P, _P, _P, _P, _I, _P, _I, _P, _P, _P, _SZ, _P]),
    "crdr_gdn_res_fwd": (_I, [C.POINTER(GdnDesc), _P, _P, _P, _P, _I, _P, _P, _SZ, _P]),
    "crdr_channel_norm_workspace": (_SZ, [C.POINTER(ChannelNormDesc)]),
    "crdr_channel_norm_fwd": (_I, [C.POINTER(ChannelNormDesc), _P, _P, _P, _P, _P, _P, _P]),
    "crdr_channel_norm_bwd": (_I, [C.POINTER(ChannelNormDesc), _P, _P, _P, _P, _P, _I, _P, _I, _P, _P, _P, _SZ, _P]),
    "crdr_instance_norm_workspace": (_SZ, [C.POINTER(InstanceNormDesc)]),
    "crdr_instance_norm_fwd": (_I, [C.POINTER(InstanceNormDesc), _P, _P, _P, _P, _P, _P, _SZ, _P]),
    "crdr_instance_norm_bwd": (_I, [C.POINTER(InstanceNormDesc), _P, _P, _P, _P, _P, _I, _P, _I, _P, _P, _P, _SZ, _P]),
    "crdr_reflect_pad_fwd": (_I, [_P, _I, _I, _I, _I, _I, _I, _I, _I, _I, _P, _I, _P]),
    "crdr_reflect_pad_bwd": (_I, [_P, _I, _I, _I, _I, _I, _I, _I, _I, _I, _P, _I, _P]),
    "crdr_pixel_shuffle_fwd": (_I, [_P, _I, _I, _I, _I, _I, _P, _I, _P]),
    "crdr_pixel_shuffle_bwd": (_I, [_P, _I, _I, _I, _I, _I, _P, _I, _P]),
    "crdr_upsample16_cat_workspace": (_SZ, [C.POINTER(Upsample16Desc)]),
    "crdr_upsample16_cat_fwd": (_I, [C.POINTER(Upsample16Desc), _P, _P, _P, _P]),
    "crdr_upsample16_cat_bwd": (_I, [C.POINTER(Upsample16Desc), _P, _P, _P, _P, _SZ, _P]),
    "crdr_gauss_symbols": (_I, [_P, _I, _P, _I, _P, _I, _P, _I, _F, _I, _I, _I, _P, _P, _P]),
    "crdr_philox_fork": (_I, [_P, _P, C.c_uint64, _P]),
    "crdr_philox_uniform": (_I, [_P, _I, _I, _I, _I, _I, _P, _I, _P]),
    "crdr_conv2d_wgrad_workspace": (_SZ, [C.POINTER(WgradDesc)]),
    "crdr_conv2d_wgrad": (_I, [C.POINTER(WgradDesc), _P, _P, _P, _P, _SZ, _P]),
    "crdr_conv2d_wgrad_partial": (_I, [C.POINTER(WgradDesc), _P, _P, _P, _P, _SZ, C.POINTER(WgradJob), _P]),
    "crdr_wgrad_reduce_batched": (_I, [_P, _P, _P, _P]),
    "crdr_pack_weight": (_I, [_P, _P, _I, _I, _I, _I, _I, _I, _P]),
    "crdr_pack_weights_batched": (_I, [_P, _P, _P, _P]),
    "crdr_epilogue_bwd_workspace": (_SZ, [C.POINTER(EbwdDesc)]),
    "crdr_epilogue_bwd": (_I, [C.POINTER(EbwdDesc), C.POINTER(EbwdIO), _P, _SZ, _P]),
    "crdr_col2im_rgb": (_I, [_P, _I, _I, _I, _I, _I, _I, _I, _I, _P, _P, _I, _I, _I, _I, _P]),
    "crdr_spectral_norm_fwd": (_I, [_P, _I, _I, _P, _P, _I, C.c_float, _P, _P, _P, _SZ, _P]),
    "crdr_spectral_norm_bwd": (_I, [_P, _P, _P, _P, _P, _I, _I, _P, _P, _SZ, _P]),
    "crdr_crop_flip_normalize": (_I, [_P, _P, _I, _I, _I, _P, _I, _P]),
    "crdr_linear_fwd": (_I, [_P, _I, _I, _I, _P, _P, _P, _I, _I, _I, _P]),
    "crdr_linear_bwd": (_I, [_P, _I, _I, _I, _P, _P, _I, _P, _I, _I, _P, _I, _P, _P, _P]),
    "crdr_linear_group_fwd": (_I, [_P, _I, _I, _I, _P, _I, _P]),
    "crdr_linear_group_bwd": (_I, [_P, _I, _I, _I, _P, _I, _P, _I, _P]),
    "crdr_affine": (_I, [_P, _I, _P, _P, _P, _I, _I64, _I, _P]),
    "crdr_colsum_workspace": (_SZ, [_I64, _I]),
    "crdr_colsum": (_I, [_P, _I, _I64, _I, _P, _I, _P, _SZ, _P]),
    "crdr_interp_ca_params": (_I, [_P, _P, _I, _I, _F, _P, _P, _P]),
    "crdr_interp_ca_params_bwd": (_I, [_P, _I, _I, _F, _P, _P, _P, _P, _P]),
    "crdr_bias_relu_slots": (_I, [_P, _I, _I64, _I, _I, _P, _P, _P]),
    "crdr_lrp": (_I, [_P, _I, _P, _I, _P, _I, _I64, _I, _P]),
    "crdr_lrp_bwd": (_I, [_P, _I, _P, _I, _P, _I, _I64, _I, _P]),
    "crdr_add_affine": (_I, [_P, _I, _P, _I, _P, _P, _P, _I, _I64, _I, _P]),
    "crdr_tanh_fwd": (_I, [_P, _I, _I64, _I, _P, _I, _P]),
    "crdr_tanh_bwd": (_I, [_P, _I, _P, _I, _I64, _I, _P, _I, _P]),
    "crdr_gauss_cond_fwd": (_I, [C.POINTER(GcDesc), _P, _P, _P, _P, _P, _P, _P, _P, _P, _P]),
    "crdr_gauss_cond_bwd": (_I, [C.POINTER(GcDesc), _P, _P, _P, _P, _P, _P, _I, _P, _P, _P, _P]),
    "crdr_entropy_bottleneck_fwd": (_I, [_P, _P, _P, _P, _I, _I, _I, _F, _P, _P, _P, _P]),
    "crdr_entropy_bottleneck_bwd": (_I, [_P, _P, _P, _I, _I, _I, _F, _P, _P, _P, _P, _P]),
    "crdr_eb_quantile_loss": (_I, [_P, _P, _P, _I, _P, _P, _P]),
    "crdr_reduce_workspace": (_SZ, [_I64]),
    "crdr_sqdiff_sum": (_I, [_P, _P, _I64, _P, _P, _SZ, _P]),
    "crdr_sqdiff_bwd": (_I, [_P, _P, _I64, _P, _F, _P, _P, _P]),
    "crdr_bce_diff_sum": (_I, [_P, _P, _I64, _F, _P, _P, _SZ, _P]),
    "crdr_bce_diff_bwd": (_I, [_P, _P, _I64, _F, _P, _F, _P, _P, _P]),
    "crdr_gan_loss_workspace": (_SZ, [_I64, _I64]),
    "crdr_gan_loss_fwd": (_I, [C.POINTER(GanLossDesc), _P, _P, _P, _P, _P, _P, _SZ, _P]),
    "crdr_gan_loss_bwd": (_I, [C.POINTER(GanLossDesc), _P, _P, _P, _P, _P, _F, _P, _P, _P, _SZ, _P]),
    "crdr_l1_sum": (_I, [_P, _P, _I64, _P, _P, _SZ, _P]),
    "crdr_l1_bwd": (_I, [_P, _P, _I64, _P, _F, _P, _P, _P]),
    "crdr_msssim_workspace": (_SZ, [_I, _I, _I, _I]),
    "crdr_msssim_fwd": (_I, [_P, _I, _P, _I, _I, _I, _I, _I, _F, _I, _P, _SZ, _I, _P, _P]),
    "crdr_msssim_bwd": (_I, [_P, _I, _P, _I, _I, _I, _I, _I, _P, _P, _P, _I, _P, _I, _P, _SZ, _P]),
    "crdr_sqnorm": (_I, [_P, _I64, _P, _P, _SZ, _P]),
    "crdr_adam_step": (_I, [_P, _P, _P, _P, _I64, _F, _F, _F, _F, _I, _P, _F, _P]),
    "crdr_adam_step_dyn": (_I, [_P, _P, _P, _P, _I64, _F, _F, _F, _P, _P, _F, _P]),
    "crdr_maxpool3s2_fwd": (_I, [_P, _P, _I, _I, _I, _I, _P]),
    "crdr_maxpool3s2_bwd": (_I, [_P, _P, _P, _I, _I, _I, _I, _P]),
    "crdr_lpips_layer_fwd": (_I, [_P, _P, _P, _I, _I, _I, _P, _P, _SZ, _P]),
    "crdr_lpips_layer_bwd": (_I, [_P, _P, _P, _I, _I, _I, _P, _P, _P]),
    "crdr_pmf_to_quantized_cdf": (_I, [_P, _I, _I, _P]),
    "crdr_rans_encode_with_indexes": (_I64, [_P, _P, _I64, _P, _I, _P, _P, _I, _P, _I64]),
    "crdr_rans_decoder_create": (_P, []),
    "crdr_rans_decoder_destroy": (None, [_P]),
    "crdr_rans_decoder_set_stream": (_I, [_P, _P, _I64]),
    "crdr_rans_decoder_decode_stream": (_I, [_P, _P, _I64, _P, _I, _P, _P, _I, _P]),
    "crdr_rans_decode_with_indexes": (_I, [_P, _I64, _P, _I64, _P, _I, _P, _P, _I, _P]),
}


class CrdrHipError(RuntimeError):
    pass


def build(force: bool = False, jobs: int = 6) -> str:
    if force:
        subprocess.run(["make", "-C", CSRC_DIR, "clean"], check=True, stdout=subprocess.DEVNULL)
    r = subprocess.run(["make", "-C", CSRC_DIR, f"-j{jobs}"], stdout=subprocess.PIPE, stderr=subprocess.STDOUT, text=True)
    if r.returncode != 0:
        raise CrdrHipError("building libcrdr_hip.so failed:\n" + r.stdout[-4000:])
    return LIB_PATH


_lock = threading.Lock()
_lib = None


def load():
    global _lib
    if _lib is not None:
        return _lib
    with _lock:
        if _lib is not None:
            return _lib
        if not os.path.exists(LIB_PATH):
            raise CrdrHipError(
                f"{LIB_PATH} not found: the HIP extension is required (run `python -c 'import __graft_entry__ as g; "
                "g.build()'` or `make -C crdr_amd/csrc`). There is no CPU fallback.")
        lib = C.CDLL(LIB_PATH)
        for name, (res, args) in SIGNATURES.items():
            fn = getattr(lib, name)
            fn.restype = res
            fn.argtypes = args
        _lib = lib
    return _lib


def check(rc, what: str = ""):
    if rc is not None and rc < 0:
        msg = load().crdr_last_error().decode("utf-8", "replace")
        raise CrdrHipError(f"{what}: rc={rc}: {msg}")
    return rc
```

crdr_amd/hip/ops.py:

```python
from __future__ import annotations

import contextlib
import ctypes as C
import os
from typing import Optional, Tuple

import torch

from . import lib as L
from . import packs, tune
from .batched import BumpArena, JobTable, SiteTables, _capturing, _require_gpu, _stream

_ws_cache = {}
_ws_keep = []
_ws_max = 0

AUTOTUNE = False
FORCED_CONV_ALGO = 0
MATRIX_BF16X3 = False
MATRIX_BF16X6 = False


def _matrix_mode() -> int:
    return 2 if MATRIX_BF16X6 else (1 if MATRIX_BF16X3 else 0)
# ... 92 lines not shown
    return ids


def _conv_trial(lib, d, ios, G: int, device, colsum: bool, trial_out):
    if trial_out is not None:
        tio, res_t, reset = ios, trial_out, None
    else:
        span = (d.N * d.OH * d.OW - 1) * d.ldy + d.OC
        res_t, reset = tune.scratch(G * span + 64, device)
        tio = (L.ConvIO * G)()
        C.memmove(tio, ios, C.sizeof(tio))
        for g in range(G):
            tio[g].y = res_t.data_ptr() + 4 * g * span
            if ios[g].pre == ios[g].y:
                tio[g].pre = tio[g].y
            if ios[g].res == ios[g].y:
                tio[g].res = tio[g].y
    keep, cost = [], 0.0

    def run(a):
        nonlocal cost
        d.reserved = a
        if colsum:
            try:
                _, _, nf = _colsum_layout(lib, d, G)
            except L.CrdrHipError:
                return False
            keep[:] = [torch.empty(G * nf, dtype=torch.float32, device=device)]
            for g in range(G):
                tio[g].cs = keep[0].data_ptr() + 4 * g * nf
        ok, cost = _tune_conv_launch(lib, d, tio, G, device)
        return ok
    return run, (lambda: res_t), reset, (lambda: cost)


def _wgrad_trial(lib, d, G: int, pa, qa, device, whole: bool):
    gsize = d.gI * d.gJ * d.kh * d.kw
    tmp = torch.zeros(G * gsize + 64, dtype=torch.float32, device=device)
    ta = (C.c_void_p * G)(*[tmp.data_ptr() + 4 * g * gsize for g in range(G)])
    jobs_t = (L.WgradJob * G)()
    d, slab = L.WgradDesc.from_buffer_copy(d), 0
    d.accumulate = 0 if whole else d.accumulate

    def run(a):
        nonlocal slab
        d.algo = _wa(a)
        nb = lib.crdr_conv2d_wgrad_grouped_workspace(C.byref(d), G)
        if nb == 0 or nb > (2 << 30):
            return False
        slab = nb
        w_, wn_ = workspace(nb, device)
        if whole:
            return lib.crdr_conv2d_wgrad(C.byref(d), pa[0], qa[0], ta[0], w_, wn_, _stream()) == 0
        return lib.crdr_conv2d_wgrad_partial_grouped(C.byref(d), pa, qa, ta, G, w_, wn_, jobs_t, _stream()) == 0
    if whole:
        return run, (lambda: tmp), None, None

    def result():
        reduce_jobs_now(jobs_t, device)
        return tmp
    return run, result, tmp.zero_, (lambda: slab / 3.8e9)


PROFILE = None


def _prof_begin():
    if PROFILE is None:
        return None
    e = torch.cuda.Event(enable_timing=True)
    e.record()
    return e


def _prof_end(kind: str, flops: float, e0, label: str = "", nbytes: float = 0.0) -> None:
    if e0 is None:
        return
    e1 = torch.cuda.Event(enable_timing=True)
    e1.record()
    PROFILE.setdefault(kind, []).append((flops, e0, e1, label, nbytes))


_WS_HEAD = 4 * 16384


def _ws_fit(key, device, need: Optional[int]) -> torch.Tensor:
    size = max(int(_ws_max * 1.25), 1 << 20)
    buf = _ws_cache.get(key)
    if buf is None or buf.numel() < (size if need is None else need):
        if need is not None and torch.cuda.is_current_stream_capturing():
            raise L.CrdrHipError("workspace must be reserved before graph capture (ops.reserve_workspace); "
                                 f"need {need} bytes, have {0 if buf is None else buf.numel()}")
        if buf is not None:
            _ws_keep.append(buf)
        buf = _ws_cache[key] = torch.zeros(size, dtype=torch.uint8, device=device)
    return buf


def workspace(nbytes: int, device, conv: bool = False) -> Tuple[int, int]:
    global _ws_max
    nbytes = int(nbytes) + (0 if conv else _WS_HEAD)
    _ws_max = max(_ws_max, nbytes)
    buf = _ws_fit((device.index if device.index is not None else torch.cuda.current_device(), _stream()), device, nbytes)
    if conv:
        return buf.data_ptr(), buf.numel()
    return buf.data_ptr() + _WS_HEAD, buf.numel() - _WS_HEAD


def reserve_workspace(device, stream: "torch.cuda.Stream") -> None:
    dev = torch.device(device)
    _ws_fit((dev.index if dev.index is not None else torch.cuda.current_device(), stream.cuda_stream), dev, None)


def _pixel_stride(t: torch.Tensor) -> int:
    n, c, h, w = t.shape
    return t.stride(3) if w > 1 else (t.stride(2) if h > 1 else (t.stride(0) if n > 1 else c))


def nhwc(t: torch.Tensor) -> Tuple[torch.Tensor, int]:
    _require_gpu(t)
    n, c, h, w = t.shape
    ld = _pixel_stride(t)
    ok = (c == 1 or t.stride(1) == 1) and ld >= c
    ok = ok and (w == 1 or t.stride(3) == ld) and (h == 1 or t.stride(2) == w * ld) and (n == 1 or t.stride(0) == h * w * ld)
    if not ok or ld % 4 != 0 or (t.data_ptr() % 16) != 0:
        if c % 4 == 0:
            t = t.contiguous(memory_format=torch.channels_last)
            if t.stride(1) != 1 or (w > 1 and t.stride(3) != c):
                t = t.permute(0, 2, 3, 1).contiguous().permute(0, 3, 1, 2)
            ld = c
        else:
            cp = (c + 3) // 4 * 4
            buf = torch.zeros((n, h, w, cp), dtype=t.dtype, device=t.device)
            buf[..., :c] = t.permute(0, 2, 3, 1)
            t = buf.permute(0, 3, 1, 2)[:, :c]
            ld = cp
    return t, ld


def dense_nhwc(t: torch.Tensor) -> torch.Tensor:
    t, ld = nhwc(t)
    if ld != t.shape[1]:
        t = t.permute(0, 2, 3, 1).contiguous().permute(0, 3, 1, 2)
    return t


def ld_for(c: int) -> int:
    return (c + 3) // 4 * 4


def empty_nhwc(n, c, h, w, device, ld: Optional[int] = None, zero: bool = False) -> torch.Tensor:
    ld = ld_for(c) if ld is None else ld
    mk = torch.zeros if (zero or ld != c) else torch.empty
    buf = mk((n, h, w, ld), dtype=torch.float32, device=device)
    return buf.permute(0, 3, 1, 2)[:, :c]


def _p(t: Optional[torch.Tensor]):
    return None if t is None else t.data_ptr()


def round32(v: int) -> int:
    return (v + 31) // 32 * 32


def pack_weight_tapmajor(w: torch.Tensor) -> torch.Tensor:
    _require_gpu(w)
    w = w.contiguous()
    I, J = w.shape[0], w.shape[1]
    T = w.shape[2] * w.shape[3]
    rows, cols = round32(I), round32(4 * T)
    dst = torch.empty((1, rows, cols), dtype=torch.float32, device=w.device)
    lib = L.load()
    L.check(lib.crdr_pack_weight(w.data_ptr(), dst.data_ptr(), I, J, T, rows, cols, 2, _stream()), "pack_weight")
    return dst


def pack_weight(w: torch.Tensor, transpose: bool) -> torch.Tensor:
    _require_gpu(w)
    w = w.contiguous()
    I, J = w.shape[0], w.shape[1]
    T = w.shape[2] * w.shape[3]
    rows, cols = (round32(J), round32(I)) if transpose else (round32(I), round32(J))
    dst = torch.empty((T, rows, cols), dtype=torch.float32, device=w.device)
# ... 465 lines not shown
```

crdr_amd/models/layer/interp_channel_attention.py:

```python
from __future__ import annotations

import math
from typing import Tuple, Union

import torch
import torch.nn as nn

from crdr_amd.hip import functional as HF


class InterpChAtt(nn.Module):
    def __init__(self, ch: int, rate_level: int, actv: str = "identity", use_interp: bool = False, use_bias: bool = False) -> None:
        super().__init__()
        if actv != "softplus" or not use_interp:
            raise NotImplementedError("CRDR uses actv=softplus, use_interp=True (config/_base_/model/*interp_ca*.yaml)")
        w = torch.ones(rate_level, 1, ch, 1, 1, dtype=torch.float32) * math.log(math.e - 1)
        self.weight = nn.Parameter(w)
        self.bias = nn.Parameter(torch.zeros(rate_level, 1, ch, 1, 1, dtype=torch.float32)) if use_bias else None
        self.use_interp, self.use_bias, self.rate_level = use_interp, use_bias, rate_level

    @staticmethod
    def _q(rate_ind: Union[float, torch.Tensor]) -> float:
        if isinstance(rate_ind, torch.Tensor):
            assert rate_ind.numel() == 1, "one rate index per batch (batch_rate_ind_sample is unsupported upstream too)"
            rate_ind = float(rate_ind.item())
        return float(rate_ind)

    def vectors(self, rate_ind) -> Tuple[torch.Tensor, torch.Tensor]:
        q = self._q(rate_ind)
        assert 0 <= q <= self.rate_level - 1, f"rate_ind = {q} should be in [0, {self.rate_level - 1}]"
        return HF.interp_ca_vectors(self.weight, self.bias, q)

    def forward(self, x, rate_ind):
        s, t = self.vectors(rate_ind)
        return HF.affine(x, s, t)
```

crdr_amd/models/subnet/autoencoder/cheng20_interpca_autoencoder.py:

```python
from __future__ import annotations

from typing import Dict

import torch.nn as nn

from crdr_amd.models.layer.hip_layers import to_image_nhwc
from crdr_amd.models.layer.interp_channel_attention import InterpChAtt
from crdr_amd.utils.registry import DECODER_REGISTRY, ENCODER_REGISTRY

from .cheng20_autoencoder import Cheng20Decoder, Cheng20Encoder


@ENCODER_REGISTRY.register()
class Cheng20InterpCaEncoder(Cheng20Encoder):
    def __init__(self, rate_level: int, in_ch: int = 3, out_ch: int = 192, main_ch: int = 192, padding_mode: str = "zeros",
                 ca_kwargs: Dict = {}, **kwargs):
        super().__init__(in_ch=in_ch, out_ch=out_ch, main_ch=main_ch, padding_mode=padding_mode)
        assert out_ch == main_ch, (f"Cheng20InterpCaEncoder: out_ch ({out_ch}) must equal main_ch ({main_ch}) -- the reference sizes the "
                                   "channel attention behind conv7 and nlam2 with main_ch")
        self.layer_list = list(self.stage_names)
        self.interp_ca_list = nn.ModuleList(InterpChAtt(main_ch, rate_level, **ca_kwargs) for _ in self.layer_list)

    def forward(self, x, rate_ind):
        x = to_image_nhwc(x)
        for name, ca in zip(self.layer_list, self.interp_ca_list):
            x = getattr(self, name)(x, affine=ca.vectors(rate_ind))
        return x


@DECODER_REGISTRY.register()
class Cheng20InterpCaDecoder(Cheng20Decoder):
    def __init__(self, rate_level: int, in_ch: int = 192, out_ch: int = 3, main_ch: int = 192, use_tanh: bool = True,
                 padding_mode: str = "zeros", ca_kwargs: Dict = {}, **kwargs):
        super().__init__(in_ch=in_ch, out_ch=out_ch, main_ch=main_ch, use_tanh=use_tanh, padding_mode=padding_mode)
        self.layer_list = list(self.stage_names)
        chans = [in_ch] * 2 + [main_ch] * (len(self.layer_list) - 2)
        self.interp_ca_list = nn.ModuleList(InterpChAtt(c, rate_level, **ca_kwargs) for c in chans)

    def forward(self, x, rate_ind):
        cas = list(self.interp_ca_list)
        x = cas[0](x, rate_ind)
        for i, name in enumerate(self.layer_list):
            nxt = cas[i + 1].vectors(rate_ind) if i + 1 < len(cas) else None
            x = getattr(self, name)(x, affine=nxt)
        return self.finish(x)
```

crdr_amd/models/subnet/autoencoder/elic_interpca_autoencoder.py:

```python
from __future__ import annotations

from typing import Dict

import torch.nn as nn

from crdr_amd.models.layer.interp_channel_attention import InterpChAtt
from crdr_amd.utils.registry import DECODER_REGISTRY, ENCODER_REGISTRY

from .elic_autoencoder import ElicDecoder, ElicEncoder
from crdr_amd.models.layer.hip_layers import to_image_nhwc


@ENCODER_REGISTRY.register()
class ElicInterpCaEncoder(ElicEncoder):
    def __init__(self, rate_level: int, in_ch: int = 3, out_ch: int = 192, main_ch: int = 192, block_mid_ch: int = 192,
                 num_blocks: int = 3, ca_kwargs: Dict = {}):
        super().__init__(in_ch=in_ch, out_ch=out_ch, main_ch=main_ch, block_mid_ch=block_mid_ch, num_blocks=num_blocks)
        chans = [main_ch] * 7 + [out_ch] * 2
        self.layer_out_ch_list = list(zip(self.stage_names, chans))
        self.interp_ca_list = nn.ModuleList(InterpChAtt(c, rate_level, **ca_kwargs) for c in chans)

    def forward(self, x, rate_ind):
        x = to_image_nhwc(x)
        for name, ca in zip(self.stage_names, self.interp_ca_list):
            x = getattr(self, name)(x, affine=ca.vectors(rate_ind))
        return x


def run_decoder_stages(dec, x, rate_ind, cond=None):
    cas = list(dec.interp_ca_list)
    x = cas[0](x, rate_ind)
    for i, name in enumerate(dec.stage_names):
        nxt = cas[i + 1].vectors(rate_ind) if i + 1 < len(cas) else None
        layer = getattr(dec, name)
        if cond is not None and name.startswith("block"):
            x = layer(x, cond, affine=nxt)
        else:
            x = layer(x, affine=nxt)
    return x


@DECODER_REGISTRY.register()
class ElicInterpCaDecoder(ElicDecoder):
    def __init__(self, rate_level: int, in_ch: int = 192, out_ch: int = 3, main_ch: int = 192, block_mid_ch: int = 192,
                 num_blocks: int = 3, use_tanh: bool = True, pixel_shuffle: bool = False, ca_kwargs: Dict = {}):
        super().__init__(in_ch=in_ch, out_ch=out_ch, main_ch=main_ch, block_mid_ch=block_mid_ch, num_blocks=num_blocks,
                         use_tanh=use_tanh, pixel_shuffle=pixel_shuffle)
        chans = [in_ch] * 2 + [main_ch] * 7
        self.layer_in_ch_list = list(zip(self.stage_names, chans))
        self.interp_ca_list = nn.ModuleList(InterpChAtt(c, rate_level, **ca_kwargs) for c in chans)

    def forward(self, x, rate_ind):
        return run_decoder_stages(self, x, rate_ind)
```

include/crdr_hip.h:

```cpp
#ifndef CRDR_HIP_H
#define CRDR_HIP_H

#include <stddef.h>
#include <stdint.h>

#ifdef __cplusplus
extern "C" {
#endif

typedef void* crdr_stream_t;

const char* crdr_last_error(void);
int crdr_version(void);
const char* crdr_arch(void);
void crdr_profile_enable(int on);
int crdr_profile_read(int kind, double* flops, double* ms, long long* launches);


#define CRDR_EPI_BIAS 1
#define CRDR_EPI_RELU 2
#define CRDR_EPI_LRELU 4
#define CRDR_EPI_VEC2 8
#define CRDR_EPI_RES 16
#define CRDR_EPI_GATE 32
#define CRDR_EPI_AFFINE 64
#define CRDR_EPI_ACCUM 128
#define CRDR_EPI_PREADD 256
#define CRDR_EPI_RELUMASK 512
#define CRDR_EPI_LRELUMASK 1024
#define CRDR_EPI_MASKOFF 2048
#define CRDR_EPI_COLSUM 4096
#define CRDR_CONV_BF16X3 16384
#define CRDR_CONV_BF16X6 32768
#define CRDR_CONV_NOSPLIT 8192

typedef struct crdr_conv_desc {
  int32_t N, H, W, C;
  int32_t OH, OW, OC;
  int32_t kh, kw, stride, pad;
  int32_t transposed;
  int32_t ldx, ldy;
  int32_t wrows, wcols;
  int32_t flags;
  int32_t ldres;
  int32_t ldg;
  int32_t wlayout;
  int32_t reserved;
  int32_t ldpre;
  int32_t ldmask;
} crdr_conv_desc;

#define CRDR_CONV_TICKETS 16384

typedef struct crdr_conv_io {
  const float* x;
  const float* w;
  float* y;
  const float* bias;
  const float* vec2;
  const float* res;
  const float* scale;
  const float* shift;
  const float* gx;
  const float* gt;
  float* sig;
  const float* pre;
  const float* mask;
  float* cs;
} crdr_conv_io;

int crdr_conv2d_num_configs(void);
int crdr_conv2d_choose_algo(const crdr_conv_desc* d, int G);
int crdr_conv2d_num_stream_configs(void);
int crdr_conv2d_num_wino_configs(void);
size_t crdr_conv2d_workspace(const crdr_conv_desc* d);
int crdr_conv2d(const crdr_conv_desc* d, const crdr_conv_io* io, void* ws, size_t ws_bytes, crdr_stream_t s);
int crdr_conv2d_colsum_layout(const crdr_conv_desc* d, int G, int* rows, int* ld);
typedef struct crdr_colsum_job {
  const float* cs;
  float* out_pre;
  float* out_post;
  int32_t rows, ld, C, accumulate;
  int32_t nslab, cpad;
  int64_t scratch_off;
} crdr_colsum_job;
int crdr_colsum_slab_rows(void);
int crdr_colsum_finish_batched(const crdr_colsum_job* jobs, const int64_t* prefix_a, const int64_t* prefix_b, const int64_t* meta,
                               float* scratch, crdr_stream_t s);

#define CRDR_MAX_GROUP 16
size_t crdr_conv2d_grouped_workspace(const crdr_conv_desc* d, int G);
int crdr_conv2d_grouped(const crdr_conv_desc* d, const crdr_conv_io* ios, int G, void* ws, size_t ws_bytes, crdr_stream_t s);
size_t crdr_conv2d_filter_cache_bytes(const crdr_conv_desc* d, int G);
typedef struct crdr_w4_filter_item {
  const float* w[16];
  float* u;
  int32_t G, Cin, Cout, wrows, wcols, kchunks, ntile, nvar;
  int32_t widx[4][9];
  int64_t units;
} crdr_w4_filter_item;
int crdr_conv2d_filter_item(const crdr_conv_desc* d, int G, crdr_w4_filter_item* item);
int crdr_w4_filters_batched(const crdr_w4_filter_item* items, const int64_t* prefix, const int64_t* meta, crdr_stream_t s);
int crdr_conv2d_grouped_ex(const crdr_conv_desc* d, const crdr_conv_io* ios, int G, void* ws, size_t ws_bytes, float* filter_cache,
                           size_t filter_cache_bytes, int filter_cache_valid, crdr_stream_t s);
double crdr_conv2d_flops(const crdr_conv_desc* d);

typedef struct crdr_wgrad_desc {
  int32_t N, PH, PW, PC, ldp;
  int32_t QH, QW, QC, ldq;
  int32_t kh, kw, stride, pad;
  int32_t gI, gJ;
  int32_t accumulate;
  int32_t algo;
} crdr_wgrad_desc;
#define CRDR_WGRAD_BF16X3 (1 << 16)
#define CRDR_WGRAD_SQUARE_Q (1 << 18)
#define CRDR_WGRAD_BF16X6 (1 << 17)
int crdr_conv2d_wgrad_num_configs(void);
int crdr_conv2d_wgrad_num_wino_configs(void);
size_t crdr_conv2d_wgrad_workspace(const crdr_wgrad_desc* d);
int crdr_conv2d_wgrad(const crdr_wgrad_desc* d, const float* p, const float* q, float* g, void* ws, size_t ws_bytes,
                      crdr_stream_t s);

typedef struct crdr_wgrad_job {
  const float* slab;
  float* g;
  int32_t PC, QC, gI, gJ, T, nsplit, smallj, accumulate;
  int32_t gJtot;
  int32_t reserved;
} crdr_wgrad_job;
int crdr_conv2d_wgrad_partial(const crdr_wgrad_desc* d, const float* p, const float* q, float* g, void* slab,
                              size_t slab_bytes, crdr_wgrad_job* job, crdr_stream_t s);
int crdr_wgrad_reduce_batched(const crdr_wgrad_job* jobs, const int64_t* prefix, const int64_t* meta, crdr_stream_t s);
size_t crdr_conv2d_wgrad_grouped_workspace(const crdr_wgrad_desc* d, int G);
int crdr_conv2d_wgrad_partial_grouped(const crdr_wgrad_desc* d, const float* const* ps, const float* const* qs,
                                      float* const* gs, int G, void* slab, size_t slab_bytes, crdr_wgrad_job* jobs,
                                      crdr_stream_t s);

int crdr_pack_weight(const float* src, float* dst, int I, int J, int T, int rows, int cols, int transpose,
                     crdr_stream_t s);

int crdr_col2im_rgb(const float* cols, int ldc, int N, int H, int W, int kh, int kw, int stride, int pad, const float* bias,
                    float* out, int ldo, int OH, int OW, int C, crdr_stream_t s);

typedef struct crdr_pack_item {
  const float* src;
  float* dst;
  int32_t I, J, T, rows, cols, mode;
  int32_t srcJ, dld;
  int64_t tstride;
} crdr_pack_item;
int crdr_pack_weights_batched(const crdr_pack_item* items, const int64_t* prefix, const int64_t* meta, crdr_stream_t s);
int crdr_pack_weight_item(const crdr_pack_item* item, crdr_stream_t s);


typedef struct crdr_ebwd_desc {
  int64_t M;
  int32_t C;
  int32_t flags;
  int32_t lddout, ldout, lddz, ldgres, ldg;
} crdr_ebwd_desc;
typedef struct crdr_ebwd_io {
  const float* dout;
  const float* out;
  const float* vec2;
  const float* scale;
  const float* shift;
  const float* gt;
  const float* sig;
  float* dz;
  float* gres;
  float* dgt;
  float* colsums;
  float* dbias_accum;
} crdr_ebwd_io;
size_t crdr_epilogue_bwd_workspace(const crdr_ebwd_desc* d);
int crdr_epilogue_bwd(const crdr_ebwd_desc* d, const crdr_ebwd_io* io, void* ws, size_t ws_bytes, crdr_stream_t s);

int crdr_spectral_norm_fwd(const float* w, int O, int K, float* u, float* v, int power_iter, float eps, float* w_out,
                           float* sigma_out, void* ws, size_t ws_bytes, crdr_stream_t s);
int crdr_spectral_norm_bwd(const float* dw_sn, const float* w, const float* u, const float* v, const float* sigma, int O, int K,
                           float* dw, void* ws, size_t ws_bytes, crdr_stream_t s);

int crdr_crop_flip_normalize(const uint8_t* pool, const int64_t* items, int N, int crop_h, int crop_w, float* out, int ldo,
                             crdr_stream_t s);

int crdr_linear_fwd(const float* x, int M, int I, int ldx, const float* w, const float* b, float* y, int O, int ldy,
                    int relu, crdr_stream_t s);
int crdr_linear_bwd(const float* x, int M, int I, int ldx, const float* w, const float* dy, int lddy, const float* y,
                    int ldy, int O, float* dx, int lddx, float* dw, float* db, crdr_stream_t s);

typedef struct crdr_linear_group {
  const float* w[CRDR_MAX_GROUP];
  const float* b[CRDR_MAX_GROUP];
  float* y[CRDR_MAX_GROUP];
  const float* dy[CRDR_MAX_GROUP];
  float* dw[CRDR_MAX_GROUP];
  float* db[CRDR_MAX_GROUP];
  int32_t O[CRDR_MAX_GROUP];
} crdr_linear_group;
int crdr_linear_group_fwd(const float* x, int M, int I, int ldx, const crdr_linear_group* g, int G, crdr_stream_t s);
int crdr_linear_group_bwd(const float* x, int M, int I, int ldx, const crdr_linear_group* g, int G, float* dx, int lddx,
                          crdr_stream_t s);

int crdr_affine(const float* x, int ldx, const float* scale, const float* shift, float* y, int ldy, int64_t M, int C,
                crdr_stream_t s);
int crdr_add_affine(const float* a, int lda, const float* r, int ldr, const float* scale, const float* shift, float* y, int ldy, int64_t M,
                    int C, crdr_stream_t s);
size_t crdr_colsum_workspace(int64_t M, int C);
int crdr_colsum(const float* x, int ldx, int64_t M, int C, float* out, int accumulate, void* ws, size_t ws_bytes,
                crdr_stream_t s);
int crdr_colsum_scatter(const float* x, int ldx, int64_t M, int C, int block, float* const* outs, int accumulate, void* ws,
                        size_t ws_bytes, crdr_stream_t s);

int crdr_interp_ca_params(const float* W, const float* B, int L, int C, float q, float* scale, float* shift,
                          crdr_stream_t s);
int crdr_interp_ca_params_bwd(const float* W, int L, int C, float q, const float* dscale, const float* dshift,
                              float* dW, float* dB, crdr_stream_t s);

int crdr_bias_relu_slots(float* a, int ld, int64_t M, int C, int n, const int32_t* c0, const float* const* bias, crdr_stream_t s);

int crdr_lrp(const float* a, int lda, const float* z, int ldz, float* y, int ldy, int64_t M, int C, crdr_stream_t s);
int crdr_lrp_bwd(const float* dy, int lddy, const float* z, int ldz, float* dz, int lddz, int64_t M, int C,
                 crdr_stream_t s);

int crdr_tanh_fwd(const float* x, int ldx, int64_t M, int C, float* y, int ldy, crdr_stream_t s);
int crdr_tanh_bwd(const float* y, int ldy, const float* dy, int lddy, int64_t M, int C, float* dx, int lddx, crdr_stream_t s);


typedef struct crdr_gc_desc {
  int32_t N;
  int32_t HW;
  int32_t C;
  int32_t ldy, ldmu, ldsigma, ldyhat;
  float scale_bound;
  float likelihood_bound;
} crdr_gc_desc;
int crdr_gauss_cond_fwd(const crdr_gc_desc* d, const float* y, const float* mu, const float* sigma, const float* noise,
                        float* yhat, float* lik_noisy, float* lik_quant, float* bits_noisy, float* bits_quant,
                        crdr_stream_t s);
int crdr_gauss_cond_bwd(const crdr_gc_desc* d, const float* y, const float* mu, const float* sigma, const float* noise,
                        const float* gbits, const float* dyhat, int lddyhat, float* dy, float* dmu, float* dsigma,
                        crdr_stream_t s);

typedef struct crdr_gc_desc2 {
  int32_t N, HW, C;
  int32_t ldy, ldmu, ldsigma, ldyhat, ldyhat2, ldnoise, ldlik, ldgrad, lddyhat;
  int32_t Ctot, c0;
  float scale_bound, likelihood_bound;
} crdr_gc_desc2;
typedef struct crdr_gc_io {
  const float *y, *mu, *sigma, *noise;
  const uint64_t* philox;
  float *yhat, *yhat2, *lik_noisy, *lik_quant, *bits_noisy, *bits_quant;
  const float *gbits, *dyhat;
  float *dy, *dmu, *dsigma;
  float* ws;
  size_t ws_bytes;
} crdr_gc_io;
size_t crdr_gauss_cond_fwd_workspace(const crdr_gc_desc2* d);
int crdr_gauss_cond_fwd2(const crdr_gc_desc2* d, const crdr_gc_io* io, crdr_stream_t s);
int crdr_gauss_cond_bwd2(const crdr_gc_desc2* d, const crdr_gc_io* io, crdr_stream_t s);
int crdr_gauss_symbols(const float* y, int ldy, const float* mu, int ldmu, const float* sigma, int ldsigma, const float* scale_table,
                       int levels, float scale_bound, int N, int HW, int C, int32_t* symbols, int32_t* indexes, crdr_stream_t s);
int crdr_philox_fork(uint64_t* state, uint64_t* call, uint64_t inc, crdr_stream_t s);
int crdr_philox_uniform(const uint64_t* philox, int N, int HW, int C, int Ctot, int c0, float* out, int ld, crdr_stream_t s);

#define CRDR_EB_PARAMS 58
int crdr_entropy_bottleneck_fwd(const float* z, const float* noise, const float* params, const float* medians, int N,
                                int HW, int C, float likelihood_bound, float* zhat, float* lik, float* bits,
                                crdr_stream_t s);
int crdr_entropy_bottleneck_bwd(const float* z, const float* noise, const float* params, int N, int HW, int C,
                                float likelihood_bound, const float* gbits, const float* dzhat, float* dz,
                                float* dparams, crdr_stream_t s);

int crdr_eb_quantile_loss(const float* quantiles, const float* params, const float* target, int C, float* loss,
                          float* dquantiles, crdr_stream_t s);

typedef struct crdr_gdn_desc {
  int64_t M;
  int32_t C, ldx, ldy, inverse;
  float beta_min, reparam_offset;
} crdr_gdn_desc;
size_t crdr_gdn_workspace(const crdr_gdn_desc* d, int backward);
int crdr_gdn_fwd(const crdr_gdn_desc* d, const float* x, const float* beta, const float* gamma, float* y, void* ws, size_t ws_bytes,
                 crdr_stream_t s);
int crdr_gdn_bwd(const crdr_gdn_desc* d, const float* x, const float* beta, const float* gamma, const float* dy, int lddy, float* dx,
                 int lddx, float* dbeta, float* dgamma, void* ws, size_t ws_bytes, crdr_stream_t s);
int crdr_gdn_res_fwd(const crdr_gdn_desc* d, const float* x, const float* beta, const float* gamma, const float* res, int ldres, float* y,
                     void* ws, size_t ws_bytes, crdr_stream_t s);

typedef struct crdr_channel_norm_desc {
  int64_t M;
  int32_t C, ldx, ldy, ldres;
  int32_t act;
  float slope, eps;
} crdr_channel_norm_desc;
size_t crdr_channel_norm_workspace(const crdr_channel_norm_desc* d);
int crdr_channel_norm_fwd(const crdr_channel_norm_desc* d, const float* x, const float* gamma, const float* beta, const float* res, float* y,
                          float* stats, crdr_stream_t s);
int crdr_channel_norm_bwd(const crdr_channel_norm_desc* d, const float* x, const float* gamma, const float* beta, const float* stats,
                          const float* dy, int lddy, float* dx, int lddx, float* dgamma, float* dbeta, void* ws, size_t ws_bytes, crdr_stream_t s);
int crdr_reflect_pad_fwd(const float* x, int N, int H, int W, int C, int ldx, int pad_l, int pad_r, int pad_t, int pad_b, float* y, int ldy,
                         crdr_stream_t s);
int crdr_reflect_pad_bwd(const float* dy, int N, int H, int W, int C, int lddy, int pad_l, int pad_r, int pad_t, int pad_b, float* dx, int lddx,
                         crdr_stream_t s);

typedef struct crdr_instance_norm_desc {
  int64_t HW;
  int32_t N, C, ldx, ldy;
  int32_t act;
  float slope, eps;
} crdr_instance_norm_desc;
size_t crdr_instance_norm_workspace(const crdr_instance_norm_desc* d);
int crdr_instance_norm_fwd(const crdr_instance_norm_desc* d, const float* x, const float* gamma, const float* beta, float* y, float* stats,
                           void* ws, size_t ws_bytes, crdr_stream_t s);
int crdr_instance_norm_bwd(const crdr_instance_norm_desc* d, const float* x, const float* gamma, const float* beta, const float* stats,
                           const float* dy, int lddy, float* dx, int lddx, float* dgamma, float* dbeta, void* ws, size_t ws_bytes, crdr_stream_t s);

int crdr_pixel_shuffle_fwd(const float* x, int ldx, int N, int H, int W, int C, float* y, int ldy, crdr_stream_t s);
int crdr_pixel_shuffle_bwd(const float* dy, int lddy, int N, int H, int W, int C, float* dx, int lddx, crdr_stream_t s);

typedef struct crdr_upsample16_desc {
  int32_t N, h, w;
  int32_t Cc;
  int32_t ldi, ldc, ldo;
  int32_t mode;
} crdr_upsample16_desc;
size_t crdr_upsample16_cat_workspace(const crdr_upsample16_desc* d);
int crdr_upsample16_cat_fwd(const crdr_upsample16_desc* d, const float* img, const float* cond, float* out, crdr_stream_t s);
int crdr_upsample16_cat_bwd(const crdr_upsample16_desc* d, const float* dout, float* dimg, float* dcond, void* ws, size_t ws_bytes,
                            crdr_stream_t s);

size_t crdr_reduce_workspace(int64_t n);
int crdr_sqdiff_sum(const float* a, const float* b, int64_t n, float* out, void* ws, size_t ws_bytes, crdr_stream_t s);
int crdr_sqdiff_bwd(const float* a, const float* b, int64_t n, const float* g, float gscale, float* da, float* db,
                    crdr_stream_t s);
int crdr_bce_diff_sum(const float* p, const float* q, int64_t n, float target, float* out, void* ws, size_t ws_bytes,
                      crdr_stream_t s);
int crdr_bce_diff_bwd(const float* p, const float* q, int64_t n, float target, const float* g, float gscale, float* dp,
                      float* dq, crdr_stream_t s);
typedef struct crdr_gan_loss_desc {
  int64_t n, nq;
  int32_t kind, center;
  float target, sgn;
} crdr_gan_loss_desc;
size_t crdr_gan_loss_workspace(int64_t n, int64_t nq);
int crdr_gan_loss_fwd(const crdr_gan_loss_desc* d, const float* p, const float* q, const float* mask, float* out, float* stats,
                      void* ws, size_t ws_bytes, crdr_stream_t s);
int crdr_gan_loss_bwd(const crdr_gan_loss_desc* d, const float* p, const float* q, const float* mask, const float* stats,
                      const float* g, float gscale, float* dp, float* dq, void* ws, size_t ws_bytes, crdr_stream_t s);
int crdr_l1_sum(const float* a, const float* b, int64_t n, float* out, void* ws, size_t ws_bytes, crdr_stream_t s);
int crdr_l1_bwd(const float* a, const float* b, int64_t n, const float* g, float gscale, float* da, float* db, crdr_stream_t s);

size_t crdr_msssim_workspace(int N, int H, int W, int which);
int crdr_msssim_fwd(const float* x, int ldx, const float* y, int ldy, int N, int H, int W, int C, float data_range, int quant,
                    float* state, size_t state_bytes, int with_maps, float* out, crdr_stream_t s);
int crdr_msssim_bwd(const float* x, int ldx, const float* y, int ldy, int N, int H, int W, int C, const float* state,
                    const float* gout, float* dx, int lddx, float* dy, int lddy, void* ws, size_t ws_bytes, crdr_stream_t s);

int crdr_sqnorm(const float* g, int64_t n, float* out, void* ws, size_t ws_bytes, crdr_stream_t s);
int crdr_adam_step(float* p, const float* g, float* m, float* v, int64_t n, float lr, float beta1, float beta2,
                   float eps, int step, const float* sqnorm, float max_norm, crdr_stream_t s);

int crdr_adam_step_dyn(float* p, const float* g, float* m, float* v, int64_t n, float beta1, float beta2, float eps,
                       const float* dyn, const float* sqnorm, float max_norm, crdr_stream_t s);

int crdr_maxpool3s2_fwd(const float* x, float* y, int N, int H, int W, int C, crdr_stream_t s);
int crdr_maxpool3s2_bwd(const float* x, const float* dy, float* dx, int N, int H, int W, int C, crdr_stream_t s);
int crdr_lpips_layer_fwd(const float* f0, const float* f1, const float* lin, int N, int HW, int C, float* out,
                         void* ws, size_t ws_bytes, crdr_stream_t s);
int crdr_lpips_layer_bwd(const float* f0, const float* f1, const float* lin, int N, int HW, int C, const float* gout,
                         float* df1, crdr_stream_t s);

int crdr_pmf_to_quantized_cdf(const float* pmf, int pmf_len, int precision, uint32_t* cdf_out);
int64_t crdr_rans_encode_with_indexes(const int32_t* symbols, const int32_t* indexes, int64_t n, const int32_t* cdfs,
                                      int cdf_stride, const int32_t* cdf_sizes, const int32_t* offsets, int ncdf,
                                      uint8_t* out, int64_t out_cap);
typedef struct crdr_rans_decoder crdr_rans_decoder;
crdr_rans_decoder* crdr_rans_decoder_create(void);
void crdr_rans_decoder_destroy(crdr_rans_decoder*);
int crdr_rans_decoder_set_stream(crdr_rans_decoder*, const uint8_t* data, int64_t nbytes);
int crdr_rans_decoder_decode_stream(crdr_rans_decoder*, const int32_t* indexes, int64_t n, const int32_t* cdfs,
                                    int cdf_stride, const int32_t* cdf_sizes, const int32_t* offsets, int ncdf,
                                    int32_t* out);
int crdr_rans_decode_with_indexes(const uint8_t* data, int64_t nbytes, const int32_t* indexes, int64_t n,
                                  const int32_t* cdfs, int cdf_stride, const int32_t* cdf_sizes,
                                  const int32_t* offsets, int ncdf, int32_t* out);

#ifdef __cplusplus
}
#endif
#endif
```

Measured before the change: 225.3 img/s.

## Batch interp-CA param kernels, fuse reduction finish in-launch, add maxpool argmax backward

Replaces the per-layer interp channel-attention parameter launches with one batched launch per encoder or decoder, forward and backward. Reductions and the gaussian-conditional bit sums now finish in the same launch through a last-arriving-block ticket, so the separate finalize kernel is dropped. Maxpool forward can record a uint8 argmax that the backward uses instead of re-reading and recomparing the input. The aim is fewer kernel launches and less memory traffic, at the cost of ticket and workspace bookkeeping plus cross-block visibility requirements on the partial sums.

```diff
diff --git a/crdr_amd/csrc/eltwise.hip b/crdr_amd/csrc/eltwise.hip
--- a/crdr_amd/csrc/eltwise.hip
+++ b/crdr_amd/csrc/eltwise.hip
@@ -3,6 +3,7 @@
 #include <cmath>
 
 #include "common.hpp"
+#include "finish.hpp"
 
 namespace crdr {
 
@@ -359,10 +360,8 @@
 
 __device__ __forceinline__ float softplusf_(float w) { return w > 20.f ? w : log1pf(expf(w)); }
 
-__global__ void interp_ca_params_kernel(const float* W, const float* B, int L, int C, float q, float* scale,
-                                        float* shift) {
-  const int c = blockIdx.x * blockDim.x + threadIdx.x;
-  if (c >= C) return;
+__device__ __forceinline__ void interp_ca_params_elem(const float* W, const float* B, int L, int C, float q, float* scale,
+                                                      float* shift, int c) {
   const float lf = floorf(q);
   const float rf = fminf(lf + 1.f, (float)(L - 1));
   const float a = rf - q;
@@ -371,11 +370,18 @@
   scale[c] = softplusf_(w);
   shift[c] = B ? B[l * C + c] * a + B[r * C + c] * (1.f - a) : 0.f;
 }
-
-__global__ void interp_ca_params_bwd_kernel(const float* W, int L, int C, float q, const float* dscale,
-                                            const float* dshift, float* dW, float* dB) {
+__global__ void interp_ca_params_kernel(const float* W, const float* B, int L, int C, float q, float* scale,
+                                        float* shift) {
   const int c = blockIdx.x * blockDim.x + threadIdx.x;
-  if (c >= C) return;
+  if (c < C) interp_ca_params_elem(W, B, L, C, q, scale, shift, c);
+}
+__global__ void interp_ca_params_batched_kernel(const crdr_interp_ca_group g, float q) {
+  const int c = blockIdx.x * blockDim.x + threadIdx.x, j = blockIdx.y;
+  if (c < g.C[j]) interp_ca_params_elem(g.W[j], g.B[j], g.L[j], g.C[j], q, g.scale[j], g.shift[j], c);
+}
+
+__device__ __forceinline__ void interp_ca_params_bwd_elem(const float* W, int L, int C, float q, const float* dscale,
+                                                          const float* dshift, float* dW, float* dB, int c) {
   const float lf = floorf(q);
   const float rf = fminf(lf + 1.f, (float)(L - 1));
   const float a = rf - q;
@@ -389,6 +395,15 @@
     dB[r * C + c] += dshift[c] * (1.f - a);
   }
 }
+__global__ void interp_ca_params_bwd_kernel(const float* W, int L, int C, float q, const float* dscale,
+                                            const float* dshift, float* dW, float* dB) {
+  const int c = blockIdx.x * blockDim.x + threadIdx.x;
+  if (c < C) interp_ca_params_bwd_elem(W, L, C, q, dscale, dshift, dW, dB, c);
+}
+__global__ void interp_ca_params_bwd_batched_kernel(const crdr_interp_ca_group g, float q) {
+  const int c = blockIdx.x * blockDim.x + threadIdx.x, j = blockIdx.y;
+  if (c < g.C[j] && g.dW[j]) interp_ca_params_bwd_elem(g.W[j], g.L[j], g.C[j], q, g.dscale[j], g.dshift[j], g.dW[j], g.dB[j], c);
+}
 
 __global__ __launch_bounds__(256) void lrp_kernel(const float* a, int lda, const float* z, int ldz, float* y, int ldy,
                                                   int64_t M, int C) {
@@ -448,10 +463,29 @@
   return r;
 }
 
+template <bool SC1>
+__device__ __forceinline__ void reduce_finish(const float* partial, int nb, float* out, float* red) {
+  float s = 0.f;
+  if (SC1) {
+    for (int e0 = threadIdx.x; e0 < nb; e0 += 1024) {
+      float x[4];
+#pragma unroll
+      for (int j = 0; j < 4; ++j) x[j] = ld_sc1(partial + min(e0 + 256 * j, nb - 1));
+#pragma unroll
+      for (int j = 0; j < 4; ++j)
+        if (e0 + 256 * j < nb) s += x[j];
+    }
+  } else {
+    for (int e = threadIdx.x; e < nb; e += 256) s += partial[e];
+  }
+  s = block_sum_256(s, red);
+  if (threadIdx.x == 0) out[0] = s;
+}
+
 enum { RED_SQDIFF = 0, RED_BCE = 1, RED_SQNORM = 2, RED_DOT = 3, RED_L1 = 4 };
 template <int OP>
 __global__ __launch_bounds__(256) void reduce_kernel(const float* a, const float* b, int64_t n, float target,
-                                                     float* partial) {
+                                                     float* partial, int* ticket, float* out) {
   __shared__ float red[4];
   float s = 0.f;
   for (int64_t e = blockIdx.x * 256ll + threadIdx.x; e < n; e += gridDim.x * 256ll) {
@@ -465,15 +499,17 @@
     }
   }
   s = block_sum_256(s, red);
-  if (threadIdx.x == 0) partial[blockIdx.x] = s;
+  if (threadIdx.x == 0) st_partial(partial + blockIdx.x, s, ticket != nullptr);
+  if (ticket) {
+    __shared__ int s_last;
+    if (finish_last_arriver(ticket, (int)gridDim.x, &s_last)) reduce_finish<true>(partial, (int)gridDim.x, out, red);
+  }
 }
 __global__ __launch_bounds__(256) void reduce_final(const float* partial, int nb, float* out) {
   __shared__ float red[4];
-  float s = 0.f;
-  for (int e = threadIdx.x; e < nb; e += 256) s += partial[e];
-  s = block_sum_256(s, red);
-  if (threadIdx.x == 0) out[0] = s;
-}
+  reduce_finish<false>(partial, nb, out, red);
+}
+static bool reduce_in_launch(int64_t n, int nb) { return nb <= 256 || n >= (int64_t)nb * 8192; }
 static int reduce_blocks(int64_t n) { return (int)std::min<int64_t>(std::max<int64_t>(cdiv64(n, 1024), 1), 1024); }
 
 __global__ __launch_bounds__(256) void sqdiff_bwd_kernel(const float* a, const float* b, int64_t n, const float* g,
@@ -566,7 +602,7 @@
   }
 }
 
-__global__ __launch_bounds__(256) void maxpool3s2_fwd_kernel(const float* x, float* y, int N, int H, int W, int C,
+__global__ __launch_bounds__(256) void maxpool3s2_fwd_kernel(const float* x, float* y, uint8_t* arg, int N, int H, int W, int C,
                                                              int OH, int OW) {
   const unsigned total = (unsigned)N * OH * OW * C;
   for (unsigned e = blockIdx.x * 256u + threadIdx.x; e < total; e += gridDim.x * 256u) {
@@ -575,13 +611,37 @@
     unsigned q = r / (unsigned)OW;
     const int ow = (int)(r - q * OW);
     const int n = (int)(q / (unsigned)OH), oh = (int)(q - (unsigned)n * OH);
-    float best = -INFINITY;
+    float best = -INFINITY, first = -INFINITY;
+    int tap = 255;
     for (int i = 0; i < 3; ++i)
       for (int j = 0; j < 3; ++j) {
         const int ih = oh * 2 + i, iw = ow * 2 + j;
-        if (ih < H && iw < W) best = fmaxf(best, x[(((int64_t)n * H + ih) * W + iw) * C + c]);
+        if (ih < H && iw < W) {
+          const float v = x[(((int64_t)n * H + ih) * W + iw) * C + c];
+          best = fmaxf(best, v);
+          if (v > first) { first = v; tap = 3 * i + j; }
+        }
       }
     y[e] = best;
+    if (arg) arg[e] = (uint8_t)tap;
+  }
+}
+__global__ __launch_bounds__(256) void maxpool3s2_bwd_arg_kernel(const uint8_t* arg, const float* dy, float* dx, int N, int H,
+                                                                 int W, int C, int OH, int OW) {
+  const unsigned total = (unsigned)N * H * W * C;
+  for (unsigned e = blockIdx.x * 256u + threadIdx.x; e < total; e += gridDim.x * 256u) {
+    unsigned r = e / (unsigned)C;
+    const int c = (int)(e - r * C);
+    unsigned q = r / (unsigned)W;
+    const int iw = (int)(r - q * W);
+    const int n = (int)(q / (unsigned)H), ih = (int)(q - (unsigned)n * H);
+    float acc = 0.f;
+    for (int oh = (ih >= 2 ? (ih - 1) / 2 : 0); oh <= ih / 2 && oh < OH; ++oh)
+      for (int ow = (iw >= 2 ? (iw - 1) / 2 : 0); ow <= iw / 2 && ow < OW; ++ow) {
+        const int64_t o = (((int64_t)n * OH + oh) * OW + ow) * C + c;
+        if ((int)arg[o] == 3 * (ih - 2 * oh) + (iw - 2 * ow)) acc += dy[o];
+      }
+    dx[e] = acc;
   }
 }
 __global__ __launch_bounds__(256) void maxpool3s2_bwd_kernel(const float* x, const float* dy, float* dx, int N, int H,
@@ -1173,6 +1233,31 @@
   CRDR_CHECK_LAUNCH("interp_ca_params_bwd");
   return 0;
 }
+extern "C" int crdr_interp_ca_params_batched(const crdr_interp_ca_group* g, int G, float q, crdr_stream_t s) {
+  CRDR_REQUIRE(g && G >= 1 && G <= CRDR_MAX_INTERP_CA, "interp_ca_params_batched: %d layers (1..%d)", G, CRDR_MAX_INTERP_CA);
+  int cmax = 0;
+  for (int j = 0; j < G; ++j) {
+    CRDR_REQUIRE(g->W[j] && g->scale[j] && g->shift[j] && g->C[j] >= 1, "interp_ca_params_batched: layer %d incomplete", j);
+    CRDR_REQUIRE(q >= 0.f && q <= (float)(g->L[j] - 1), "interp_ca_params_batched: rate_ind %f outside [0, %d] (layer %d)", q, g->L[j] - 1, j);
+    cmax = std::max(cmax, (int)g->C[j]);
+  }
+  hipLaunchKernelGGL(interp_ca_params_batched_kernel, dim3(cdiv(cmax, 64), G), dim3(64), 0, as_stream(s), *g, q);
+  CRDR_CHECK_LAUNCH("interp_ca_params_batched");
+  return 0;
+}
+extern "C" int crdr_interp_ca_params_bwd_batched(const crdr_interp_ca_group* g, int G, float q, crdr_stream_t s) {
+  CRDR_REQUIRE(g && G >= 1 && G <= CRDR_MAX_INTERP_CA, "interp_ca_params_bwd_batched: %d layers (1..%d)", G, CRDR_MAX_INTERP_CA);
+  int cmax = 0;
+  for (int j = 0; j < G; ++j) {
+    if (!g->dW[j]) continue;
+    CRDR_REQUIRE(g->W[j] && g->dscale[j] && (!g->dB[j] || g->dshift[j]) && g->C[j] >= 1, "interp_ca_params_bwd_batched: layer %d incomplete", j);
+    cmax = std::max(cmax, (int)g->C[j]);
+  }
+  if (!cmax) return 0;
+  hipLaunchKernelGGL(interp_ca_params_bwd_batched_kernel, dim3(cdiv(cmax, 64), G), dim3(64), 0, as_stream(s), *g, q);
+  CRDR_CHECK_LAUNCH("interp_ca_params_bwd_batched");
+  return 0;
+}
 
 extern "C" int crdr_lrp(const float* a, int lda, const float* z, int ldz, float* y, int ldy, int64_t M, int C,
                         crdr_stream_t s) {
@@ -1258,15 +1343,17 @@
   return 0;
 }
 
-extern "C" size_t crdr_reduce_workspace(int64_t n) { return (size_t)reduce_blocks(n) * sizeof(float); }
+extern "C" size_t crdr_reduce_workspace(int64_t n) { return (size_t)reduce_blocks(n) * sizeof(float) + kFinishTicketBytes; }
 
 template <int OP>
 static int run_reduce(const float* a, const float* b, int64_t n, float target, float* out, void* ws, size_t ws_bytes,
                       crdr_stream_t s, const char* what) {
   const int nb = reduce_blocks(n);
   CRDR_REQUIRE(a && out && ws_bytes >= (size_t)nb * sizeof(float), "%s: bad arguments", what);
-  hipLaunchKernelGGL(reduce_kernel<OP>, dim3(nb), dim3(256), 0, as_stream(s), a, b, n, target, (float*)ws);
+  int* ticket = reduce_in_launch(n, nb) ? finish_tickets(ws, ws_bytes, (size_t)nb * sizeof(float)) : nullptr;
+  hipLaunchKernelGGL(reduce_kernel<OP>, dim3(nb), dim3(256), 0, as_stream(s), a, b, n, target, (float*)ws, ticket, out);
   CRDR_CHECK_LAUNCH(what);
+  if (ticket) return 0;
   hipLaunchKernelGGL(reduce_final, dim3(1), dim3(256), 0, as_stream(s), (const float*)ws, nb, out);
   CRDR_CHECK_LAUNCH(what);
   return 0;
@@ -1298,8 +1385,9 @@
   float* part = (float*)ws;
   float* dot = part + nb;
   hipStream_t st = as_stream(s);
-  hipLaunchKernelGGL(reduce_kernel<RED_DOT>, dim3(nb), dim3(256), 0, st, dw_sn, w, n, 0.f, part);
-  hipLaunchKernelGGL(reduce_final, dim3(1), dim3(256), 0, st, (const float*)part, nb, dot);
+  int* ticket = reduce_in_launch(n, nb) ? finish_tickets(ws, ws_bytes, (size_t)(nb + 1) * sizeof(float)) : nullptr;
+  hipLaunchKernelGGL(reduce_kernel<RED_DOT>, dim3(nb), dim3(256), 0, st, dw_sn, w, n, 0.f, part, ticket, dot);
+  if (!ticket) hipLaunchKernelGGL(reduce_final, dim3(1), dim3(256), 0, st, (const float*)part, nb, dot);
   hipLaunchKernelGGL(sn_bwd_kernel, dim3(grid_for(n)), dim3(256), 0, st, dw_sn, u, v, sigma, (const float*)dot, O, K, dw);
   CRDR_CHECK_LAUNCH("spectral_norm_bwd");
   return 0;
@@ -1373,9 +1461,28 @@
   CRDR_REQUIRE(x && y && H >= 3 && W >= 3, "maxpool: bad arguments");
   CRDR_REQUIRE((long long)N * H * W * C < (1ll << 31), "maxpool: %lld elements (32-bit element index)", (long long)N * H * W * C);
   const int OH = (H - 3) / 2 + 1, OW = (W - 3) / 2 + 1;
-  hipLaunchKernelGGL(maxpool3s2_fwd_kernel, dim3(grid_for((int64_t)N * OH * OW * C)), dim3(256), 0, as_stream(s), x, y, N,
-                     H, W, C, OH, OW);
+  hipLaunchKernelGGL(maxpool3s2_fwd_kernel, dim3(grid_for((int64_t)N * OH * OW * C)), dim3(256), 0, as_stream(s), x, y,
+                     (uint8_t*)nullptr, N, H, W, C, OH, OW);
   CRDR_CHECK_LAUNCH("maxpool_fwd");
+  return 0;
+}
+extern "C" int crdr_maxpool3s2_fwd_argmax(const float* x, float* y, uint8_t* argmax, int N, int H, int W, int C, crdr_stream_t s) {
+  CRDR_REQUIRE(x && y && argmax && H >= 3 && W >= 3, "maxpool_fwd_argmax: bad arguments");
+  CRDR_REQUIRE((long long)N * H * W * C < (1ll << 31), "maxpool_fwd_argmax: %lld elements (32-bit element index)", (long long)N * H * W * C);
+  const int OH = (H - 3) / 2 + 1, OW = (W - 3) / 2 + 1;
+  hipLaunchKernelGGL(maxpool3s2_fwd_kernel, dim3(grid_for((int64_t)N * OH * OW * C)), dim3(256), 0, as_stream(s), x, y, argmax, N, H,
+                     W, C, OH, OW);
+  CRDR_CHECK_LAUNCH("maxpool_fwd_argmax");
+  return 0;
+}
+extern "C" int crdr_maxpool3s2_bwd_argmax(const uint8_t* argmax, const float* dy, float* dx, int N, int H, int W, int C,
+                                          crdr_stream_t s) {
+  CRDR_REQUIRE(argmax && dy && dx && H >= 3 && W >= 3, "maxpool_bwd_argmax: bad arguments");
+  CRDR_REQUIRE((long long)N * H * W * C < (1ll << 31), "maxpool_bwd_argmax: %lld elements (32-bit element index)", (long long)N * H * W * C);
+  const int OH = (H - 3) / 2 + 1, OW = (W - 3) / 2 + 1;
+  hipLaunchKernelGGL(maxpool3s2_bwd_arg_kernel, dim3(grid_for((int64_t)N * H * W * C)), dim3(256), 0, as_stream(s), argmax, dy, dx,
+                     N, H, W, C, OH, OW);
+  CRDR_CHECK_LAUNCH("maxpool_bwd_argmax");
   return 0;
 }
 extern "C" int crdr_maxpool3s2_bwd(const float* x, const float* dy, float* dx, int N, int H, int W, int C,
diff --git a/crdr_amd/csrc/entropy.hip b/crdr_amd/csrc/entropy.hip
--- a/crdr_amd/csrc/entropy.hip
+++ b/crdr_amd/csrc/entropy.hip
@@ -3,6 +3,7 @@
 #include <cmath>
 
 #include "common.hpp"
+#include "finish.hpp"
 
 namespace crdr {
 
@@ -109,8 +110,37 @@
   }
 }
 
+template <bool SC1>
+__device__ __forceinline__ void gauss_cond_finish(const float* part, int B, float* bits_noisy, float* bits_quant, int n, float* red) {
+  float sn = 0.f, sq = 0.f;
+  if (SC1) {
+    for (int b0 = threadIdx.x; b0 < B; b0 += 2048) {
+      float xn[8], xq[8];
+#pragma unroll
+      for (int j = 0; j < 8; ++j) {
+        const float* v = part + ((size_t)n * B + min(b0 + 256 * j, B - 1)) * 2;
+        xn[j] = ld_sc1(v); xq[j] = ld_sc1(v + 1);
+      }
+#pragma unroll
+      for (int j = 0; j < 8; ++j)
+        if (b0 + 256 * j < B) { sn += xn[j]; sq += xq[j]; }
+    }
+  } else {
+    for (int b = threadIdx.x; b < B; b += 256) {
+      const float2 v = *reinterpret_cast<const float2*>(part + ((size_t)n * B + b) * 2);
+      sn += v.x; sq += v.y;
+    }
+  }
+  sn = block_sum(sn, red);
+  sq = block_sum(sq, red);
+  if (threadIdx.x == 0) {
+    if (bits_noisy) bits_noisy[n] += sn;
+    if (bits_quant) bits_quant[n] += sq;
+  }
+}
+
 template <bool VEC>
-__global__ __launch_bounds__(256) void gauss_cond_fwd_kernel(const GcArgs p, float* part) {
+__global__ __launch_bounds__(256) void gauss_cond_fwd_kernel(const GcArgs p, float* part, int* tickets) {
   __shared__ float red[16];
   const int n = blockIdx.y, C = p.d.C;
   const int per_img = p.d.HW * C;
@@ -165,28 +195,22 @@
   if (threadIdx.x == 0) {
     if (part) {
       float* o = part + ((size_t)n * gridDim.x + blockIdx.x) * 2;
-      o[0] = sn; o[1] = sq;
+      st_partial(o, sn, tickets != nullptr); st_partial(o + 1, sq, tickets != nullptr);
     } else {
       if (p.io.bits_noisy && noisy) p.io.bits_noisy[n] += sn;
       if (p.io.bits_quant) p.io.bits_quant[n] += sq;
     }
   }
+  if (tickets) {
+    __shared__ int s_last;
+    if (finish_last_arriver(tickets + n, (int)gridDim.x, &s_last))
+      gauss_cond_finish<true>(part, (int)gridDim.x, noisy ? p.io.bits_noisy : nullptr, p.io.bits_quant, n, red);
+  }
 }
 
 __global__ __launch_bounds__(256) void gauss_cond_finish_kernel(const float* part, int B, float* bits_noisy, float* bits_quant) {
   __shared__ float red[16];
-  const int n = blockIdx.x;
-  float sn = 0.f, sq = 0.f;
-  for (int b = threadIdx.x; b < B; b += 256) {
-    const float2 v = *reinterpret_cast<const float2*>(part + ((size_t)n * B + b) * 2);
-    sn += v.x; sq += v.y;
-  }
-  sn = block_sum(sn, red);
-  sq = block_sum(sq, red);
-  if (threadIdx.x == 0) {
-    if (bits_noisy) bits_noisy[n] += sn;
-    if (bits_quant) bits_quant[n] += sq;
-  }
+  gauss_cond_finish<false>(part, B, bits_noisy, bits_quant, blockIdx.x, red);
 }
 
 __device__ __forceinline__ void gc_elem_bwd(const GcArgs& p, float yv, float m, float sraw, float u, float gb, float ste, float& gy_out,
@@ -492,7 +516,7 @@
 
 extern "C" size_t crdr_gauss_cond_fwd_workspace(const crdr_gc_desc2* d) {
   if (!d) return 0;
-  return (size_t)d->N * gc_blocks(d) * 2 * sizeof(float);
+  return (size_t)d->N * gc_blocks(d) * 2 * sizeof(float) + kFinishTicketBytes;
 }
 
 extern "C" int crdr_gauss_cond_fwd2(const crdr_gc_desc2* d, const crdr_gc_io* io, crdr_stream_t s) {
@@ -511,16 +535,18 @@
                    ((!io->lik_noisy && !io->lik_quant) || (g.ldlik % 4 == 0 && al16(io->lik_noisy) && al16(io->lik_quant)));
   int B = gc_blocks(d);
   float* part = io->ws;
-  if (!part || io->ws_bytes < crdr_gauss_cond_fwd_workspace(d) || !(io->bits_noisy || io->bits_quant)) {
+  const size_t part_bytes = (size_t)d->N * B * 2 * sizeof(float);
+  if (!part || io->ws_bytes < part_bytes || !(io->bits_noisy || io->bits_quant)) {
     part = nullptr;
     if (io->bits_noisy || io->bits_quant) B = 1;
   }
+  int* tickets = part && d->N <= kFinishTickets ? finish_tickets(part, io->ws_bytes, part_bytes) : nullptr;
   if (vec)
-    hipLaunchKernelGGL(gauss_cond_fwd_kernel<true>, dim3(B, d->N), dim3(256), 0, as_stream(s), a, part);
+    hipLaunchKernelGGL(gauss_cond_fwd_kernel<true>, dim3(B, d->N), dim3(256), 0, as_stream(s), a, part, tickets);
   else
-    hipLaunchKernelGGL(gauss_cond_fwd_kernel<false>, dim3(B, d->N), dim3(256), 0, as_stream(s), a, part);
+    hipLaunchKernelGGL(gauss_cond_fwd_kernel<false>, dim3(B, d->N), dim3(256), 0, as_stream(s), a, part, tickets);
   CRDR_CHECK_LAUNCH("gauss_cond_fwd");
-  if (part) {
+  if (part && !tickets) {
     const bool noisy = io->noise || io->philox;
     hipLaunchKernelGGL(gauss_cond_finish_kernel, dim3(d->N), dim3(256), 0, as_stream(s), part, B, noisy ? io->bits_noisy : nullptr,
                        io->bits_quant);
diff --git a/crdr_amd/csrc/finish.hpp b/crdr_amd/csrc/finish.hpp
--- /dev/null
+++ b/crdr_amd/csrc/finish.hpp
@@ -0,0 +1,40 @@
+#pragma once
+#include "common.hpp"
+
+namespace crdr {
+
+constexpr int kFinishTickets = CRDR_FINISH_TICKETS;
+constexpr size_t kFinishTicketBytes = (size_t)kFinishTickets * sizeof(int) + 16;
+
+static inline int* finish_tickets(void* ws, size_t ws_bytes, size_t data_bytes) {
+  if (!ws || ws_bytes < data_bytes + kFinishTicketBytes) return nullptr;
+  const uintptr_t end = (reinterpret_cast<uintptr_t>(ws) + ws_bytes) & ~uintptr_t(15);
+  return reinterpret_cast<int*>(end - (size_t)kFinishTickets * sizeof(int));
+}
+
+
+__device__ __forceinline__ void st_sc1(float* p, float v) { __hip_atomic_store(p, v, __ATOMIC_RELAXED, __HIP_MEMORY_SCOPE_AGENT); }
+__device__ __forceinline__ float ld_sc1(const float* p) {
+  return __hip_atomic_load(const_cast<float*>(p), __ATOMIC_RELAXED, __HIP_MEMORY_SCOPE_AGENT);
+}
+__device__ __forceinline__ void st_partial(float* p, float v, bool sc1) {
+  if (sc1) st_sc1(p, v); else *p = v;
+}
+__device__ __forceinline__ bool finish_last_arriver(int* ticket, int n, int* s_flag) {
+  asm volatile("s_waitcnt vmcnt(0)" ::: "memory");
+  __syncthreads();
+  if (threadIdx.x == 0) {
+    const int t = __hip_atomic_fetch_add(ticket, 1, __ATOMIC_RELAXED, __HIP_MEMORY_SCOPE_AGENT);
+    const int last = t == n - 1;
+    if (last) {
+      __hip_atomic_store(ticket, 0, __ATOMIC_RELAXED, __HIP_MEMORY_SCOPE_AGENT);
+      __builtin_amdgcn_fence(__ATOMIC_ACQUIRE, "agent");
+      asm volatile("s_waitcnt vmcnt(0)" ::: "memory");
+    }
+    *s_flag = last;
+  }
+  __syncthreads();
+  return *s_flag != 0;
+}
+
+}
diff --git a/crdr_amd/hip/functional.py b/crdr_amd/hip/functional.py
--- a/crdr_amd/hip/functional.py
+++ b/crdr_amd/hip/functional.py
@@ -331,6 +331,65 @@
     return _InterpCaVectors.apply(W, B, float(q))
 
 
+class _InterpCaVectorsGroup(torch.autograd.Function):
+
+    @staticmethod
+    def forward(ctx, q: float, n: int, *wb):
+        lib = L.load()
+        Ws, Bs = wb[:n], wb[n:]
+        g = L.InterpCaGroup()
+        outs = []
+        for j, (W, B) in enumerate(zip(Ws, Bs)):
+            Cc = W.shape[2]
+            scale = torch.empty(Cc, dtype=torch.float32, device=W.device)
+            shift = torch.empty(Cc, dtype=torch.float32, device=W.device)
+            g.W[j], g.B[j], g.L[j], g.C[j] = W.data_ptr(), None if B is None else B.data_ptr(), W.shape[0], Cc
+            g.scale[j], g.shift[j] = scale.data_ptr(), shift.data_ptr()
+            outs += [scale, shift]
+        L.check(lib.crdr_interp_ca_params_batched(C.byref(g), n, float(q), ops._stream()), "interp_ca_params_batched")
+        ctx.q, ctx.n = float(q), n
+        ctx.Bs = Bs
+        ctx.save_for_backward(*Ws)
+        return tuple(outs)
+
+    @staticmethod
+    def backward(ctx, *grads):
+        Ws, n = ctx.saved_tensors, ctx.n
+        lib = L.load()
+        g = L.InterpCaGroup()
+        ret_w, ret_b, keep = [None] * n, [None] * n, []
+        for j, W in enumerate(Ws):
+            B = ctx.Bs[j]
+            need_w, need_b = ctx.needs_input_grad[2 + j], B is not None and ctx.needs_input_grad[2 + n + j]
+            direct = W.is_leaf and (B is None or B.is_leaf)
+            if direct:
+                dW = grad_slot(W) if need_w else None
+                dB = grad_slot(B) if need_b else None
+            else:
+                dW = ret_w[j] = torch.zeros_like(W)
+                dB = ret_b[j] = torch.zeros_like(W) if B is not None else None
+            if dW is None and dB is None:
+                continue
+            if dW is None:
+                dW = torch.zeros_like(W)
+            dscale, dshift = grads[2 * j].contiguous(), grads[2 * j + 1].contiguous()
+            keep += [dW, dscale, dshift]
+            g.W[j], g.L[j], g.C[j] = W.data_ptr(), W.shape[0], W.shape[2]
+            g.dscale[j], g.dshift[j] = dscale.data_ptr(), dshift.data_ptr()
+            g.dW[j], g.dB[j] = dW.data_ptr(), None if dB is None else dB.data_ptr()
+        L.check(lib.crdr_interp_ca_params_bwd_batched(C.byref(g), n, ctx.q, ops._stream()), "interp_ca_params_bwd_batched")
+        return (None, None, *ret_w, *ret_b)
+
+
+def interp_ca_vectors_group(params, q: float):
+    out = []
+    for i in range(0, len(params), L.MAX_INTERP_CA):
+        part = params[i:i + L.MAX_INTERP_CA]
+        v = _InterpCaVectorsGroup.apply(float(q), len(part), *[w for w, _ in part], *[b for _, b in part])
+        out += [(v[2 * j], v[2 * j + 1]) for j in range(len(part))]
+    return out
+
+
 class _Affine(torch.autograd.Function):
     @staticmethod
     def forward(ctx, x, scale, shift):
@@ -776,18 +835,23 @@
         n, c, h, w = x.shape
         oh, ow = (h - 3) // 2 + 1, (w - 3) // 2 + 1
         y = ops.empty_nhwc(n, c, oh, ow, x.device, ld=c)
-        L.check(lib.crdr_maxpool3s2_fwd(x.data_ptr(), y.data_ptr(), n, h, w, c, ops._stream()), "maxpool_fwd")
-        ctx.save_for_backward(x)
+        if not ctx.needs_input_grad[0]:
+            L.check(lib.crdr_maxpool3s2_fwd(x.data_ptr(), y.data_ptr(), n, h, w, c, ops._stream()), "maxpool_fwd")
+            return y
+        arg = torch.empty(n * oh * ow * c, dtype=torch.uint8, device=x.device)
+        L.check(lib.crdr_maxpool3s2_fwd_argmax(x.data_ptr(), y.data_ptr(), arg.data_ptr(), n, h, w, c, ops._stream()), "maxpool_fwd_argmax")
+        ctx.save_for_backward(arg)
+        ctx.shape = (n, c, h, w)
         return y
 
     @staticmethod
     def backward(ctx, dy):
-        (x,) = ctx.saved_tensors
-        lib = L.load()
-        n, c, h, w = x.shape
+        (arg,) = ctx.saved_tensors
+        lib = L.load()
+        n, c, h, w = ctx.shape
         dy = ops.dense_nhwc(dy)
-        dx = ops.empty_nhwc(n, c, h, w, x.device, ld=c)
-        L.check(lib.crdr_maxpool3s2_bwd(x.data_ptr(), dy.data_ptr(), dx.data_ptr(), n, h, w, c, ops._stream()), "maxpool_bwd")
+        dx = ops.empty_nhwc(n, c, h, w, arg.device, ld=c)
+        L.check(lib.crdr_maxpool3s2_bwd_argmax(arg.data_ptr(), dy.data_ptr(), dx.data_ptr(), n, h, w, c, ops._stream()), "maxpool_bwd_argmax")
         return dx
 
 
diff --git a/crdr_amd/hip/lib.py b/crdr_amd/hip/lib.py
--- a/crdr_amd/hip/lib.py
+++ b/crdr_amd/hip/lib.py
@@ -47,6 +47,14 @@
 
 class LinearGroup(C.Structure):
     _fields_ = [(n, c_void_p * 16) for n in ("w", "b", "y", "dy", "dw", "db")] + [("O", C.c_int32 * 16)]
+
+
+MAX_INTERP_CA = 16
+
+
+class InterpCaGroup(C.Structure):
+    _fields_ = [(n, c_void_p * MAX_INTERP_CA) for n in ("W", "B", "scale", "shift", "dscale", "dshift", "dW", "dB")] + [
+        ("L", C.c_int32 * MAX_INTERP_CA), ("C", C.c_int32 * MAX_INTERP_CA)]
 
 
 class PackItem(C.Structure):
@@ -184,6 +192,8 @@
     "crdr_colsum": (_I, [_P, _I, _I64, _I, _P, _I, _P, _SZ, _P]),
     "crdr_interp_ca_params": (_I, [_P, _P, _I, _I, _F, _P, _P, _P]),
     "crdr_interp_ca_params_bwd": (_I, [_P, _I, _I, _F, _P, _P, _P, _P, _P]),
+    "crdr_interp_ca_params_batched": (_I, [C.POINTER(InterpCaGroup), _I, _F, _P]),
+    "crdr_interp_ca_params_bwd_batched": (_I, [C.POINTER(InterpCaGroup), _I, _F, _P]),
     "crdr_bias_relu_slots": (_I, [_P, _I, _I64, _I, _I, _P, _P, _P]),
     "crdr_lrp": (_I, [_P, _I, _P, _I, _P, _I, _I64, _I, _P]),
     "crdr_lrp_bwd": (_I, [_P, _I, _P, _I, _P, _I, _I64, _I, _P]),
@@ -213,6 +223,8 @@
     "crdr_adam_step_dyn": (_I, [_P, _P, _P, _P, _I64, _F, _F, _F, _P, _P, _F, _P]),
     "crdr_maxpool3s2_fwd": (_I, [_P, _P, _I, _I, _I, _I, _P]),
     "crdr_maxpool3s2_bwd": (_I, [_P, _P, _P, _I, _I, _I, _I, _P]),
+    "crdr_maxpool3s2_fwd_argmax": (_I, [_P, _P, _P, _I, _I, _I, _I, _P]),
+    "crdr_maxpool3s2_bwd_argmax": (_I, [_P, _P, _P, _I, _I, _I, _I, _P]),
     "crdr_lpips_layer_fwd": (_I, [_P, _P, _P, _I, _I, _I, _P, _P, _SZ, _P]),
     "crdr_lpips_layer_bwd": (_I, [_P, _P, _P, _I, _I, _I, _P, _P, _P]),
     "crdr_pmf_to_quantized_cdf": (_I, [_P, _I, _I, _P]),
diff --git a/crdr_amd/hip/ops.py b/crdr_amd/hip/ops.py
--- a/crdr_amd/hip/ops.py
+++ b/crdr_amd/hip/ops.py
@@ -198,6 +198,7 @@
 
 
 _WS_HEAD = 4 * 16384
+_WS_TAIL = 4 * 256 + 16
 
 
 def _ws_fit(key, device, need: Optional[int]) -> torch.Tensor:
@@ -215,7 +216,7 @@
 
 def workspace(nbytes: int, device, conv: bool = False) -> Tuple[int, int]:
     global _ws_max
-    nbytes = int(nbytes) + (0 if conv else _WS_HEAD)
+    nbytes = int(nbytes) + (0 if conv else _WS_HEAD) + _WS_TAIL
     _ws_max = max(_ws_max, nbytes)
     buf = _ws_fit((device.index if device.index is not None else torch.cuda.current_device(), _stream()), device, nbytes)
     if conv:
diff --git a/crdr_amd/models/layer/interp_channel_attention.py b/crdr_amd/models/layer/interp_channel_attention.py
--- a/crdr_amd/models/layer/interp_channel_attention.py
+++ b/crdr_amd/models/layer/interp_channel_attention.py
@@ -31,6 +31,14 @@
         assert 0 <= q <= self.rate_level - 1, f"rate_ind = {q} should be in [0, {self.rate_level - 1}]"
         return HF.interp_ca_vectors(self.weight, self.bias, q)
 
+    @staticmethod
+    def vectors_of(cas, rate_ind):
+        cas = list(cas)
+        q = InterpChAtt._q(rate_ind)
+        for ca in cas:
+            assert 0 <= q <= ca.rate_level - 1, f"rate_ind = {q} should be in [0, {ca.rate_level - 1}]"
+        return HF.interp_ca_vectors_group([(ca.weight, ca.bias) for ca in cas], q)
+
     def forward(self, x, rate_ind):
         s, t = self.vectors(rate_ind)
         return HF.affine(x, s, t)
diff --git a/crdr_amd/models/subnet/autoencoder/cheng20_interpca_autoencoder.py b/crdr_amd/models/subnet/autoencoder/cheng20_interpca_autoencoder.py
--- a/crdr_amd/models/subnet/autoencoder/cheng20_interpca_autoencoder.py
+++ b/crdr_amd/models/subnet/autoencoder/cheng20_interpca_autoencoder.py
@@ -4,6 +4,7 @@
 
 import torch.nn as nn
 
+from crdr_amd.hip import functional as HF
 from crdr_amd.models.layer.hip_layers import to_image_nhwc
 from crdr_amd.models.layer.interp_channel_attention import InterpChAtt
 from crdr_amd.utils.registry import DECODER_REGISTRY, ENCODER_REGISTRY
@@ -23,8 +24,9 @@
 
     def forward(self, x, rate_ind):
         x = to_image_nhwc(x)
-        for name, ca in zip(self.layer_list, self.interp_ca_list):
-            x = getattr(self, name)(x, affine=ca.vectors(rate_ind))
+        vecs = InterpChAtt.vectors_of(self.interp_ca_list, rate_ind)
+        for name, affine in zip(self.layer_list, vecs):
+            x = getattr(self, name)(x, affine=affine)
         return x
 
 
@@ -38,9 +40,9 @@
         self.interp_ca_list = nn.ModuleList(InterpChAtt(c, rate_level, **ca_kwargs) for c in chans)
 
     def forward(self, x, rate_ind):
-        cas = list(self.interp_ca_list)
-        x = cas[0](x, rate_ind)
+        vecs = InterpChAtt.vectors_of(self.interp_ca_list, rate_ind)
+        x = HF.affine(x, *vecs[0])
         for i, name in enumerate(self.layer_list):
-            nxt = cas[i + 1].vectors(rate_ind) if i + 1 < len(cas) else None
+            nxt = vecs[i + 1] if i + 1 < len(vecs) else None
             x = getattr(self, name)(x, affine=nxt)
         return self.finish(x)
diff --git a/crdr_amd/models/subnet/autoencoder/elic_interpca_autoencoder.py b/crdr_amd/models/subnet/autoencoder/elic_interpca_autoencoder.py
--- a/crdr_amd/models/subnet/autoencoder/elic_interpca_autoencoder.py
+++ b/crdr_amd/models/subnet/autoencoder/elic_interpca_autoencoder.py
@@ -4,6 +4,7 @@
 
 import torch.nn as nn
 
+from crdr_amd.hip import functional as HF
 from crdr_amd.models.layer.interp_channel_attention import InterpChAtt
 from crdr_amd.utils.registry import DECODER_REGISTRY, ENCODER_REGISTRY
 
@@ -22,16 +23,17 @@
 
     def forward(self, x, rate_ind):
         x = to_image_nhwc(x)
-        for name, ca in zip(self.stage_names, self.interp_ca_list):
-            x = getattr(self, name)(x, affine=ca.vectors(rate_ind))
+        vecs = InterpChAtt.vectors_of(self.interp_ca_list, rate_ind)
+        for name, affine in zip(self.stage_names, vecs):
+            x = getattr(self, name)(x, affine=affine)
         return x
 
 
 def run_decoder_stages(dec, x, rate_ind, cond=None):
-    cas = list(dec.interp_ca_list)
-    x = cas[0](x, rate_ind)
+    vecs = InterpChAtt.vectors_of(dec.interp_ca_list, rate_ind)
+    x = HF.affine(x, *vecs[0])
     for i, name in enumerate(dec.stage_names):
-        nxt = cas[i + 1].vectors(rate_ind) if i + 1 < len(cas) else None
+        nxt = vecs[i + 1] if i + 1 < len(vecs) else None
         layer = getattr(dec, name)
         if cond is not None and name.startswith("block"):
             x = layer(x, cond, affine=nxt)
diff --git a/include/crdr_hip.h b/include/crdr_hip.h
--- a/include/crdr_hip.h
+++ b/include/crdr_hip.h
@@ -51,6 +51,8 @@
 } crdr_conv_desc;
 
 #define CRDR_CONV_TICKETS 16384
+
+#define CRDR_FINISH_TICKETS 256
 
 typedef struct crdr_conv_io {
   const float* x;
@@ -217,6 +219,21 @@
                           crdr_stream_t s);
 int crdr_interp_ca_params_bwd(const float* W, int L, int C, float q, const float* dscale, const float* dshift,
                               float* dW, float* dB, crdr_stream_t s);
+#define CRDR_MAX_INTERP_CA 16
+typedef struct crdr_interp_ca_group {
+  const float* W[CRDR_MAX_INTERP_CA];
+  const float* B[CRDR_MAX_INTERP_CA];
+  float* scale[CRDR_MAX_INTERP_CA];
+  float* shift[CRDR_MAX_INTERP_CA];
+  const float* dscale[CRDR_MAX_INTERP_CA];
+  const float* dshift[CRDR_MAX_INTERP_CA];
+  float* dW[CRDR_MAX_INTERP_CA];
+  float* dB[CRDR_MAX_INTERP_CA];
+  int32_t L[CRDR_MAX_INTERP_CA];
+  int32_t C[CRDR_MAX_INTERP_CA];
+} crdr_interp_ca_group;
+int crdr_interp_ca_params_batched(const crdr_interp_ca_group* g, int G, float q, crdr_stream_t s);
+int crdr_interp_ca_params_bwd_batched(const crdr_interp_ca_group* g, int G, float q, crdr_stream_t s);
 
 int crdr_bias_relu_slots(float* a, int ld, int64_t M, int C, int n, const int32_t* c0, const float* const* bias, crdr_stream_t s);
 
@@ -368,6 +385,8 @@
 
 int crdr_maxpool3s2_fwd(const float* x, float* y, int N, int H, int W, int C, crdr_stream_t s);
 int crdr_maxpool3s2_bwd(const float* x, const float* dy, float* dx, int N, int H, int W, int C, crdr_stream_t s);
+int crdr_maxpool3s2_fwd_argmax(const float* x, float* y, uint8_t* argmax, int N, int H, int W, int C, crdr_stream_t s);
+int crdr_maxpool3s2_bwd_argmax(const uint8_t* argmax, const float* dy, float* dx, int N, int H, int W, int C, crdr_stream_t s);
 int crdr_lpips_layer_fwd(const float* f0, const float* f1, const float* lin, int N, int HW, int C, float* out,
                          void* ws, size_t ws_bytes, crdr_stream_t s);
 int crdr_lpips_layer_bwd(const float* f0, const float* f1, const float* lin, int N, int HW, int C, const float* gout,
```

After: 226.0 img/s (median of 6 runs). Within noise of the previous version (+0.3%).
